# noegroup/bgflow

Hardware: AMD Instinct MI355X
Metric: flow samples/s (fwd+log|detJ|) at batch 2^20 (higher is better)
Workload: dtype f32 (split-f16 conditioner GEMMs: hi+lo f16 operand pairs, f32 accumulate)

## Files before the change

bgflow_amd/_lib.py:

```python
import ctypes
import os

import torch

_HERE = os.path.dirname(os.path.abspath(__file__))
LIB_PATH = os.environ.get("BGK_LIB") or os.path.join(_HERE, "libbgflow_amd.so")
_lib = None

i32, i64, f32, f64, vp = ctypes.c_int32, ctypes.c_int64, ctypes.c_float, ctypes.c_double, ctypes.c_void_p

_SIGNATURES = {
    "bgk_abi_version": (ctypes.c_int, []),
    "bgk_last_error": (ctypes.c_char_p, []),
    "bgk_set_option": (ctypes.c_int, [i32, i32]),
    "bgk_detmath_probe": (ctypes.c_int, [vp, i64, i32, vp, vp]),
    "bgk_rqs_transform": (ctypes.c_int, [vp, i64, vp, i64, i32, vp, i64, i32, i32, i32,
                                         f64, f64, f64, f64, f64, f64, f64, i32,
                                         vp, i64, vp, i32, vp, vp, vp]),
    "bgk_rqs_backward": (ctypes.c_int, [vp, i64, vp, i64, i32, vp, i64, i32, i32, i32,
                                        f64, f64, f64, f64, f64, f64, f64, i32,
                                        vp, i64, vp, vp, i64, vp, i64, vp, i32, vp]),
    "bgk_affine_transform": (ctypes.c_int, [vp, i64, vp, i64, vp, i64, vp, i32, i32, i32, i64, i32,
                                            vp, i64, vp, i32, vp]),
    "bgk_affine_backward": (ctypes.c_int, [vp, i64, vp, i64, vp, i64, vp, i32, i32, i32, i64, i32,
                                           vp, i64, vp, vp, i64, vp, i64, vp, i64, vp, vp, vp, vp]),
    "bgk_coupling_affine_dense_h2_train": (ctypes.c_int, [vp, vp, vp, i32, i32, vp, vp, vp, vp, i32, vp, vp, vp, vp, i32,
                                                          vp, i32, i32, i32, vp, i64, i64, i32, vp, i64, vp, i32,
                                                          vp, vp, vp, vp, i64, vp, vp, i64, vp]),
    "bgk_mlp_backward_dx": (ctypes.c_int, [vp, i64, i32, vp, vp, i64, vp, i64, i32, i32, vp, vp, vp, vp, i32, i64,
                                           vp, vp, vp, vp, vp, i64, vp, i64, vp, vp, vp]),
    "bgk_pack_mlp_h2": (ctypes.c_int, [vp, vp, i32, i32, vp, vp, i32, vp, vp, i32, vp, i32, i32, i32, vp, vp, vp, vp, vp]),
    "bgk_pack_mlp_h2_many": (ctypes.c_int, [i32] + [vp] * 18 + [vp]),
    "bgk_coupling_affine_dense_fwd64_train": (ctypes.c_int, [vp, i64, i32, vp, vp, vp, vp, i32, vp, vp, vp, vp, i32,
                                                             vp, i32, i32, i32, vp, i64, i64, i32, vp, i64, vp, i32,
                                                             vp, vp, vp, vp, vp, vp, i64, vp]),
    "bgk_pack_mlp_h2_t": (ctypes.c_int, [vp, i32, i32, vp, i32, vp, i32, vp, vp, vp, vp, vp]),
    "bgk_pack_mlp_h2_t_many": (ctypes.c_int, [i32] + [vp] * 11 + [vp]),
    "bgk_mlp_weight_grad_workspace": (i64, [i64, i32, i32, i32, i32]),
    "bgk_mlp_weight_grad": (ctypes.c_int, [vp, i64, i32, vp, vp, vp, vp, i64, i32, i32, i32, vp, i64, i32, i32, i64, vp, i64,
                                           vp, vp, vp, vp, vp, vp, i32, vp, vp]),
    "bgk_mlp_weight_grad_reduce_many": (ctypes.c_int, [i32] + [vp] * 12 + [i32, vp]),
    "bgk_ic_xyz2ic": (ctypes.c_int, [vp, i64, vp, i32, vp, i32, i32, f32, i32, vp, vp, i32, f32, i64,
                                     vp, vp, vp, i64, vp, i64, vp, i32, vp, vp]),
    "bgk_ic_ic2xyz": (ctypes.c_int, [vp, vp, vp, i64, vp, i64, vp, i32, vp, i32, i32, f32, i32,
                                     vp, vp, i32, f32, i64, vp, i64, vp, i32, vp, vp]),
    "bgk_ic_refsys": (ctypes.c_int, [vp, i64, i32, i32, f32, i32, vp, vp, i32, vp]),
    "bgk_icdf_ic2xyz": (ctypes.c_int, [vp, vp, vp, i64, vp, i64, vp, vp, vp, vp, i32, f32, vp, i32, vp, i32, i32, f32, i32,
                                       vp, vp, i32, f32, i64, vp, i64, vp, i32, vp, vp]),
    "bgk_icdf_ic2xyz_reg": (ctypes.c_int, [vp, vp, vp, vp, vp, i32, f32, vp, i32, vp, i32, f32, i32, vp, vp, i32, f64, i64,
                                           vp, i64, vp, i32, vp, vp]),
    "bgk_icdf_ic2xyz_uni": (ctypes.c_int, [vp, vp, vp, vp, vp, i32, f32, vp, i32, vp, i32, f32, i32, vp, vp, i32, f64, i64,
                                           vp, i64, vp, i32, vp, vp]),
    "bgk_icdf_ic2xyz_uni_train": (ctypes.c_int, [vp, vp, vp, vp, vp, i32, f32, vp, i32, vp, i32, f32, i32, vp, vp, i32, f64, i64,
                                                 vp, i64, vp, i32, vp, vp, vp, vp, vp, vp]),
    "bgk_icdf_ic2xyz_uni_train_kl": (ctypes.c_int, [vp, vp, vp, vp, vp, i32, f32, vp, i32, vp, i32, f32, i32, vp, vp, i32, f64, i64,
                                                    vp, i64, vp, vp, vp, vp, vp, vp, vp, f64, f64, f64, i32, vp, vp, vp, vp, vp]),
    "bgk_xyz2ic_cdf_uni": (ctypes.c_int, [vp, vp, i32, f32, vp, i32, vp, i32, f32, i32, vp, vp, i32, f64, i64,
                                          vp, vp, vp, vp, vp, i32, vp, vp]),
    "bgk_ic_ic2xyz_backward": (ctypes.c_int, [vp, vp, vp, i64, vp, i64, vp, i32, vp, i32, i32, f32, i32, vp, i32, i64,
                                              vp, i64, vp, vp, vp, vp, i64, vp, i64, vp, vp]),
    "bgk_cdf_transform": (ctypes.c_int, [vp, i64, vp, i64, i32, i32, i32, f32, vp, i64, vp, i32, vp]),
    "bgk_cdf_backward": (ctypes.c_int, [vp, i64, vp, i64, vp, i64, i32, i32, i32, f32, vp, i64, vp, vp, i64, vp]),
    "bgk_ic_xyz2ic_backward": (ctypes.c_int, [vp, i64, vp, i32, vp, i32, i32, f32, i32, vp, i32, i64,
                                              vp, vp, vp, i64, vp, i64, vp, vp, i64, vp]),
    "bgk_ic_refsys_backward": (ctypes.c_int, [vp, vp, vp, i64, i32, i32, f32, i32, vp, vp]),
    "bgk_coupling_rqs_dense": (ctypes.c_int, [vp, i64, i32, i32, vp, vp, vp, i32, i32, i32,
                                              vp, i64, i64, i32, i32, ctypes.c_uint64, i32,
                                              f64, f64, f64, f64, f64, f64, f64, i32,
                                              vp, i64, vp, i32, vp, vp, vp]),
    "bgk_coupling_rqs_dense_h2": (ctypes.c_int, [vp, i64, i32, i32, vp, vp, vp, f32, f32, f32, vp, i32, i32, i32, i32,
                                                 vp, i64, i64, i32, i32, ctypes.c_uint64, i32,
                                                 f64, f64, f64, f64, f64, f64, f64, i32,
                                                 vp, i64, vp, i32, vp, vp, vp]),
    "bgk_coupling_rqs_dense_deep": (ctypes.c_int, [vp, i64, i32, i32, vp, vp, vp, f32, vp, f32, i32, i32,
                                                   vp, i64, i64, i32, i32, ctypes.c_uint64, i32,
                                                   f64, f64, f64, f64, f64, f64, f64, i32,
                                                   vp, i64, vp, i32, vp, vp, vp]),
    "bgk_coupling_rqs_dense_h2_mc": (ctypes.c_int, [vp, vp, vp, i32, i32, vp, vp, vp, f32, f32, f32, vp, i32, i32, i32, i32,
                                                    vp, i64, i64, i32, i32, ctypes.c_uint64, i32,
                                                    f64, f64, f64, f64, f64, f64, f64, i32,
                                                    vp, i64, vp, i32, vp, vp, vp]),
    "bgk_coupling_affine_dense_h2_mc": (ctypes.c_int, [vp, vp, vp, i32, i32,
                                                       vp, vp, vp, f32, f32, f32, i32, vp, vp, vp, f32, f32, f32, i32,
                                                       i32, vp, i32, i32, i32, vp, i64, i64, i32, vp, i64, vp, i32, vp]),
    "bgk_coupling_affine_dense_h3_mc": (ctypes.c_int, [vp, vp, vp, i32, i32,
                                                       vp, vp, vp, vp, f32, f32, f32, f32, i32, vp, vp, vp, vp, f32, f32, f32, f32, i32,
                                                       i32, vp, i32, i32, i32, vp, i64, i64, i32, vp, i64, vp, i32, vp]),
    "bgk_pack_dense_h2": (ctypes.c_int, [vp, vp, i32, i32, vp, vp, vp, vp, i32, vp, i32, i32, i32, vp, vp, vp, vp, vp]),
    "bgk_coupling_rqs_dense_h2_train": (ctypes.c_int, [vp, i64, i32, i32, vp, vp, vp, f32, f32, f32, vp, i32, i32, i32,
                                                       vp, i64, i64, i32, i32, ctypes.c_uint64, i32,
                                                       f64, f64, f64, f64, f64, f64, f64, i32,
                                                       vp, i64, vp, i32, vp, vp, vp, vp, i64, vp, i32, vp]),
    "bgk_coupling_rqs_dense_h2_backward": (ctypes.c_int, [vp, vp, f32, vp, i32, i32, vp, i64, i64, i32, i32, i32, ctypes.c_uint64, i32,
                                                          f64, f64, f64, f64, f64, f64, f64, i32,
                                                          vp, i64, vp, vp, i64, vp, i64, vp, vp]),
    "bgk_coupling_affine_dense_h2": (ctypes.c_int, [vp, i64, i32, i32,
                                                    vp, vp, vp, f32, f32, f32, i32, vp, vp, vp, f32, f32, f32, i32,
                                                    i32, vp, i32, i32, i32, vp, i64, i64, i32, vp, i64, vp, i32, vp]),
    "bgk_coupling_affine_dense_h3": (ctypes.c_int, [vp, i64, i32, i32,
                                                    vp, vp, vp, vp, f32, f32, f32, f32, i32, vp, vp, vp, vp, f32, f32, f32, f32, i32,
                                                    i32, vp, i32, i32, i32, vp, i64, i64, i32, vp, i64, vp, i32, vp]),
    "bgk_coupling_affine_dense_deep": (ctypes.c_int, [vp, i64, i32, i32,
                                                      vp, vp, vp, f32, vp, f32, i32, vp, vp, vp, f32, vp, f32, i32,
                                                      i32, i32, vp, i32, i32, i32, vp, i64, i64, i32, vp, i64, vp, i32, vp]),
    "bgk_pack_dense_h2_t": (ctypes.c_int, [vp, i32, vp, vp, i32, vp, vp, vp, vp, vp]),
    "bgk_dense_backward_dx": (ctypes.c_int, [vp, i64, i32, vp, vp, vp, i64, i32, i32, vp, vp, vp, vp, i32, i64,
                                             vp, vp, vp, vp, vp, i64, vp, i64, vp, vp, vp]),
    "bgk_dense_weight_grad_reduce_many": (ctypes.c_int, [i32] + [vp] * 10 + [i32, vp]),
    "bgk_pack_dense_h2_many": (ctypes.c_int, [i32] + [vp] * 14 + [vp]),
    "bgk_pack_dense_h2_t_many": (ctypes.c_int, [i32] + [vp] * 9 + [vp]),
    "bgk_column_sum": (ctypes.c_int, [vp, i64, i64, i32, vp, i32, vp, vp]),
    "bgk_absmax": (ctypes.c_int, [vp, i64, i64, i32, vp, vp]),
    "bgk_whiten": (ctypes.c_int, [vp, i64, vp, vp, vp, i32, i32, i64, vp, i64, vp]),
    "bgk_normal_energy": (ctypes.c_int, [vp, i64, vp, i32, i64, f64, f64, vp, vp]),
    "bgk_normal_energy_backward": (ctypes.c_int, [vp, i64, vp, i32, i64, f64, vp, vp, i64, vp]),
    "bgk_energy_fields": (ctypes.c_int, [vp, vp, vp, vp, vp, vp, i32, i64, f64, f64, f64, vp, vp, i32, vp, i32, vp, vp]),
    "bgk_energy_fields_backward": (ctypes.c_int, [vp, vp, vp, vp, vp, vp, i32, i64, f64, vp, vp, vp, vp, i32, vp, vp, vp, vp]),
    "bgk_philox_fields": (ctypes.c_int, [ctypes.c_uint64, ctypes.c_uint32, i64, i32, vp, vp, vp, vp, vp, vp, vp, vp, f64, i64, vp, vp]),
    "bgk_colmap": (ctypes.c_int, [vp, i32, vp, i32, vp, vp, ctypes.c_uint64, ctypes.c_uint32, i64, i64, vp, i32, f64, vp, vp]),
    "bgk_grad_nan_flag":(ctypes.c_int, [vp, i64, vp, vp]),
    "bgk_adam_step": (ctypes.c_int, [vp, vp, vp, vp, i64, f32, f32, f32, f32, f32, i64, vp, vp, vp]),
    "bgk_dense_weight_grad_workspace": (i64, [i64, i32, i32]),
    "bgk_dense_weight_grad": (ctypes.c_int, [vp, i64, i32, vp, vp, vp, vp, i32, vp, i64, i32, i32, i64, vp, i64,
                                             vp, vp, vp, vp, vp, vp, i32, vp, vp]),
    "bgk_pack_rqs_columns": (i32, [i32, i32, vp, vp]),
    "bgk_dense_layer": (ctypes.c_int, [vp, i64, i64, i32, vp, i32, f32, vp, vp, i32, i32, vp, i64, i32, vp]),
    "bgk_pack_linear_layer": (ctypes.c_int, [vp, i64, i32, i32, vp, vp, vp]),
    "bgk_dense_layer_steps": (ctypes.c_int, [i32]),
    "bgk_refresh_linear_layer": (ctypes.c_int, [vp, i64, i32, i32, i32, vp, vp, vp, vp]),
    "bgk_activation": (ctypes.c_int, [vp, i64, i64, i32, i32, vp, i64, vp]),
    "bgk_activation_backward": (ctypes.c_int, [vp, i64, vp, i64, i64, i32, i32, vp, i64, vp]),
    "bgk_affine_net_backward64_workspace": (i64, [i64, i32, i32, i32, i32]),
    "bgk_affine_net_backward64": (ctypes.c_int, [vp, i64, i32, vp, vp, vp, i64, i32, i32, i32, vp, vp, vp, vp, i32, i64,
                                                 vp, i64, vp, i64, vp, vp, i64, vp, vp, vp, vp, vp, vp, i32, vp]),
    "bgk_affine_coupling_backward64_workspace": (i64, [i64, i32, i32, i32, i32, i32, i32]),
    "bgk_affine_coupling_backward64": (ctypes.c_int, [vp, i64, i32, vp, i64, i32, vp, i64, vp,
                                                      vp, vp, vp, vp, vp, i64,
                                                      vp, vp, vp, vp, vp, vp, i32, i32, i32,
                                                      vp, vp, vp, vp, vp, vp, vp, i32, i32, i32,
                                                      vp, i32, i64, vp, i64, vp, vp, i64, vp, i64, vp, vp, i64, vp, vp, i32, vp]),
    "bgk_linear_weight_grad_workspace": (i64, [i64, i32, i32]),
    "bgk_linear_weight_grad": (ctypes.c_int, [vp, i64, i32, vp, i64, i32, i64, vp, i64, vp, vp, i32, vp, vp]),
}

ABI_SYMBOLS = tuple(_SIGNATURES)


def lib():
    global _lib
    if _lib is None:
        if not os.path.exists(LIB_PATH):
            raise RuntimeError(
                f"{LIB_PATH} is missing: the MI355X kernels are not built. Run `python -m bgflow_amd.build` "
                "(hipcc, gfx950). bgflow_amd has no CPU fallback.")
        try:
            handle = ctypes.CDLL(LIB_PATH)
        except OSError as e:
            raise RuntimeError(f"cannot load {LIB_PATH}: {e}. bgflow_amd has no CPU fallback.") from e
        for name, (res, args) in _SIGNATURES.items():
            fn = getattr(handle, name)
            fn.restype = res
            fn.argtypes = args
        _lib = handle
    return _lib


def check(status, what):
    if status != 0:
        msg = lib().bgk_last_error().decode(errors="replace")
        if status == -1 and "Minimal bin" in msg:
            raise ValueError(msg)
        raise RuntimeError(f"{what} failed (status {status}): {msg}")


def require_hip(*tensors):
    for t in tensors:
        if t is None:
            continue
        if not t.is_cuda:
            raise RuntimeError(
                "bgflow_amd kernels run on MI355X (HIP) tensors only; got a tensor on "
                f"'{t.device}'. There is no CPU fallback in this package.")
        if t.dtype not in (torch.float32, torch.int32):
            raise RuntimeError(f"bgflow_amd kernels are float32; got {t.dtype}")


def ptr(t):
    return None if t is None else ctypes.c_void_p(t.data_ptr())


def cond_segments(parts):
    rows = [rowmajor(t) for t in parts]
    n = len(rows)
    ptrs = (ctypes.c_void_p * n)(*[t.data_ptr() for t, _ in rows])
    lds = (ctypes.c_int64 * n)(*[ld for _, ld in rows])
    widths = (ctypes.c_int32 * n)(*[t.shape[1] for t, _ in rows])
    return ptrs, lds, widths, n, rows


def stream_ptr(device=None):
    return ctypes.c_void_p(torch.cuda.current_stream(device).cuda_stream)


def rowmajor(t):
    assert t.dim() == 2, "expected [batch, features]"
    if t.stride(1) != 1 and t.shape[1] > 1:
        t = t.contiguous()
    if t.shape[1] == 1 and t.stride(1) != 1:
        t = t.contiguous()
    ld = t.stride(0) if t.shape[0] > 1 else t.shape[1]
    if t.shape[0] > 1 and ld < t.shape[1]:
        t = t.contiguous()
        ld = t.stride(0)
    return t, ld
```

bgflow_amd/csrc/bgk_capi.hip:

```cpp
#include <stdarg.h>

#include "bgk_common.h"
#include "bgk_fused2.h"

extern int bgk_affine_variant;

static thread_local char g_err[512] = "";

void bgk_set_error(const char* fmt, ...) {
    va_list ap;
    va_start(ap, fmt);
    vsnprintf(g_err, sizeof(g_err), fmt, ap);
    va_end(ap);
}

extern "C" int bgk_abi_version(void) { return 1; }
extern "C" const char* bgk_last_error(void) { return g_err; }

extern "C" int bgk_set_option(int32_t option, int32_t value) {
    if (option == 1 && (value == 1 || value == 2)) {
        const int prev = bgk_h2_variant;
        bgk_h2_variant = value;
        return prev;
    }
    if (option == 2 && (value == 1 || value == 2)) {
        const int prev = bgk_affine_variant;
        bgk_affine_variant = value;
        return prev;
    }
    if (option == 3 && (value == 1 || value == 2)) {
        const int prev = bgk_rc_vjp_variant;
        bgk_rc_vjp_variant = value;
        return prev;
    }
    bgk_set_error("bgk_set_option: unknown option %d / value %d", option, value);
    return BGK_EINVAL;
}

namespace {
__global__ void detmath_probe_kernel(const float* x, int64_t n, int which, float* out) {
    int64_t i = (int64_t)blockIdx.x * blockDim.x + threadIdx.x;
    if (i >= n) return;
    float v = x[i], r;
    switch (which) {
        case 0: r = bgk_expf(v); break;
        case 1: r = bgk_logf(v); break;
        case 2: r = bgk_softplusf(v, 0.69384102162f); break;
        case 3: r = bgk_siluf(v); break;
        case 4: r = bgk_tanhf(v); break;
        default: r = v;
    }
    out[i] = r;
}
}

extern "C" int bgk_detmath_probe(const float* x, int64_t n, int32_t which, float* out, void* stream) {
    if (n <= 0) return 0;
    int grid = (int)((n + 255) / 256);
    hipLaunchKernelGGL(detmath_probe_kernel, dim3(grid), dim3(256), 0, (hipStream_t)stream, x, n, which, out);
    return bgk_launch_status("bgk_detmath_probe");
}
```

bgflow_amd/csrc/bgk_fused2.h:

```cpp
#ifndef BGK_FUSED2_H
#define BGK_FUSED2_H
#include <stdint.h>

#define BGK_MAX_COND 3
struct BgkCondSegs { const float* ptr[BGK_MAX_COND]; int64_t ld[BGK_MAX_COND]; int32_t w[BGK_MAX_COND]; int32_t n; };

int bgk_launch_rqs_dense_h2v2(const char* what, const float* cond, int64_t ldc, int32_t d_c, int32_t periodic,
                              const void* A0p, const void* A1p, const void* A2p, float c0, float c1, float c2, const float* cs_dev,
                              int32_t act, const float* y, int64_t ldy, int64_t B, int32_t d, uint64_t circ_mask, int32_t inverse,
                              double left, double right, double bottom, double top,
                              double min_bin_width, double min_bin_height, double min_derivative, int32_t identity_init,
                              float* out, int64_t ldo, float* dlogp, int32_t accumulate, int32_t* bin_idx, int32_t* oob_count,
                              void* stream, const BgkCondSegs* segs = nullptr);

int bgk_launch_rqs_dense_h2v2_train(const char* what, float* z0, float* z1, float* params, int64_t ldp, const int32_t* src_col,
                                    const float* cond, int64_t ldc, int32_t d_c, int32_t periodic,
                                    const void* A0p, const void* A1p, const void* A2p, float c0, float c1, float c2, const float* cs_dev,
                                    int32_t act, const float* y, int64_t ldy, int64_t B, int32_t d, uint64_t circ_mask, int32_t inverse,
                                    double left, double right, double bottom, double top,
                                    double min_bin_width, double min_bin_height, double min_derivative, int32_t identity_init,
                                    float* out, int64_t ldo, float* dlogp, int32_t accumulate, int32_t* bin_idx, int32_t* oob_count,
                                    void* stream, const BgkCondSegs* segs = nullptr);

int bgk_launch_rqs_bwd_recompute(const char* what, const float* z1, const void* A2p, float c2, const float* cs_dev, int32_t act,
                                 const float* y, int64_t ldy, int64_t B, int32_t d, uint64_t circ_mask, int32_t inverse,
                                 double left, double right, double bottom, double top,
                                 double min_bin_width, double min_bin_height, double min_derivative, int32_t identity_init,
                                 const float* g_out, int64_t ldgo, const float* g_dlogp, float* g_y, int64_t ldgy,
                                 float* g_params, int64_t ldgp, float* g_absmax, void* stream);

int bgk_launch_rqs_dense_h2v2_bf16(const char* what, const float* cond, int64_t ldc, int32_t d_c, int32_t periodic,
                                   const void* A0p, const void* A1p, const void* A2p, float c0, float c1, float c2, const float* cs_dev,
                                   int32_t act, const float* y, int64_t ldy, int64_t B, int32_t d, uint64_t circ_mask, int32_t inverse,
                                   double left, double right, double bottom, double top,
                                   double min_bin_width, double min_bin_height, double min_derivative, int32_t identity_init,
                                   float* out, int64_t ldo, float* dlogp, int32_t accumulate, int32_t* bin_idx, int32_t* oob_count,
                                   void* stream, const BgkCondSegs* segs = nullptr);

int bgk_launch_affine_dense_v2(const float* cond, int64_t ldc, int32_t d_c, int32_t periodic,
                               const void* sA0, const void* sA1, const void* sA1b, const void* sA2, float sc0, float sc1, float sc1b, float sc2, int32_t s_act,
                               const void* tA0, const void* tA1, const void* tA1b, const void* tA2, float tc0, float tc1, float tc1b, float tc2, int32_t t_act,
                               const float* log_alpha, int32_t preserve_volume, int32_t is_circular, int32_t inverse,
                               const float* y, int64_t ldy, int64_t B, int32_t d,
                               float* out, int64_t ldo, float* dlogp, int32_t accumulate, void* stream, const BgkCondSegs* segs = nullptr);

struct BgkAffTrainSave { const float* s_cs; float* s_z0; float* s_z1; const float* t_cs; float* t_z0; float* t_z1; float* mu; float* s_raw; int64_t ldms;
                         int64_t ldz; };
int bgk_launch_affine_dense_v2_train(const BgkAffTrainSave* save, const float* cond, int64_t ldc, int32_t d_c, int32_t periodic,
                               const void* sA0, const void* sA1, const void* sA1b, const void* sA2, float sc0, float sc1, float sc1b, float sc2, int32_t s_act,
                               const void* tA0, const void* tA1, const void* tA1b, const void* tA2, float tc0, float tc1, float tc1b, float tc2, int32_t t_act,
                               const float* log_alpha, int32_t preserve_volume, int32_t is_circular, int32_t inverse,
                               const float* y, int64_t ldy, int64_t B, int32_t d,
                               float* out, int64_t ldo, float* dlogp, int32_t accumulate, void* stream, const BgkCondSegs* segs = nullptr);

extern int bgk_h2_variant;
extern int bgk_rc_vjp_variant;

#endif
```

bgflow_amd/csrc/bgk_fused2.hip:

```cpp
#include "bgk_common.h"
#include "bgk_fused2.h"

#ifndef BGK_V2_SAVE
#define BGK_V2_SAVE 0
#endif
#if BGK_V2_SAVE
#include "bgk_mfma_h2.h"
#include "bgk_rqs_vjp.h"
#define coupling_rqs_dense_h2v2_kernel coupling_rqs_dense_h2v2_train_kernel
#endif
#ifndef BGK_V2_BF16
#define BGK_V2_BF16 0
#endif
#if BGK_V2_BF16
#define coupling_rqs_dense_h2v2_kernel coupling_rqs_dense_h2v2_bf16_kernel
typedef short s16x8 __attribute__((ext_vector_type(8)));
#endif
#ifndef BGK_V2_AFFTRAIN
#define BGK_V2_AFFTRAIN 0
#endif
#if BGK_V2_AFFTRAIN
#define coupling_affine_dense_v2_kernel coupling_affine_dense_v2_train_kernel
#endif
constexpr int NPROD = BGK_V2_BF16 ? 1 : 3;

namespace {

typedef float f32x16 __attribute__((ext_vector_type(16)));
typedef _Float16 h16x8 __attribute__((ext_vector_type(8)));
typedef unsigned u32x4 __attribute__((ext_vector_type(4)));

constexpr int FW = 4;
constexpr int FTHREADS = FW * 64;
constexpr int KB = 8;
constexpr int PPD = 3 * KB + 1;
constexpr int DPC = 128 / PPD;
constexpr int SROW = 33;
constexpr int ST = BGK_V2_SAVE ? 33 : 32;
constexpr int KS = 8;
constexpr int GBLK = KS * 8 + 4;
#ifndef BGK_V2_KARG
#define BGK_V2_KARG 2
#endif
#ifndef BGK_V2_RD
#define BGK_V2_RD 4
#endif
#ifndef BGK_V2_TS
#define BGK_V2_TS 0
#endif
#if BGK_V2_TS
#define V2_TS(k) do { const unsigned long long t_ = __builtin_amdgcn_s_memtime(); if (lane == 0 && a.bin_idx) a.bin_idx[b0 * d + (k)] = (int)(unsigned)t_; } while (0)
#else
#define V2_TS(k) do { } while (0)
#endif
constexpr int RD = BGK_V2_RD;
constexpr int EH = 34;

struct CondSegs {
    const float* ptr[BGK_MAX_COND]; int64_t ld[BGK_MAX_COND]; int w[BGK_MAX_COND]; int off[BGK_MAX_COND]; uint32_t magic[BGK_MAX_COND];
    int n;
};

struct SetK { float gnum, low, high, dstep; float kc[7]; };

struct SpC {
    float left, right;
    SetK sa, sb;
    float beta, kout, min_d;
};

struct V2Args {
    CondSegs cs;
    int d_c; int periodic;
    const float* y; int64_t ldy; float* out; int64_t ldo; int d; uint32_t magic_d;
    int64_t B; float* dlogp; int accumulate; int32_t* bin_idx; int32_t* oob_count;
    const uint4* A0; const uint4* A1; const uint4* A2; int S0; int n_chunks; int last_tiles;
    float c0, c1, c2; const float* cs_dev;
    uint64_t circ_mask;
    SpC sc;
    int lds_per_wave;
    int nfs, ys, stage, y_dma, out_lin;
#if BGK_V2_SAVE
    float* z0; float* z1;
    float* params; int64_t ldp;
    const int32_t* src_col;
#endif
};
typedef const __attribute__((address_space(4))) V2Args* kargs_t;

struct BFrag { h16x8 hi[KS], lo[KS]; };
struct TFrag { u32x4 hi, lo; };

__device__ __forceinline__ int drow(int m, int r, int hh) { return 32 * m + (r & 3) + 8 * (r >> 2) + 4 * hh; }

template <int NT, int MS = 4, int RDX = RD>
struct Live {
    static constexpr int NTS = KS * NT;
    static constexpr int NEV = NPROD * NTS + NT;
    f32x16 (&out)[4];
    const BFrag& b;
    const uint4* W;
    unsigned voff;
    TFrag (&ring)[RDX];
    __amdgpu_buffer_rsrc_t rs;

    template <int BLK>
    __device__ __forceinline__ u32x4 blk() {
        return __builtin_amdgcn_raw_buffer_load_b128(rs, voff + ((BLK * 1024) & 4095), (BLK * 1024) & ~4095, 0);
    }
    template <int T>
    __device__ __forceinline__ void load() {
        if constexpr (T < NTS) {
            constexpr int s = T / NT, m = T % NT;
#if BGK_V2_BF16
            ring[T % RDX].hi = blk<(s * MS + m) * 2>();
#else
            ring[T % RDX].hi = blk<(s * MS + m) * 2>();
            ring[T % RDX].lo = blk<(s * MS + m) * 2 + 1>();
#endif
        } else if constexpr (T < NTS + NT) {
            ring[T % RDX].hi = blk<KS * MS * 2 + (T - NTS)>();
        }
    }
    template <int T0, int T1>
    __device__ __forceinline__ void loads() {
        if constexpr (T0 < T1) { load<T0>(); loads<T0 + 1, T1>(); }
    }
    __device__ __forceinline__ void start() {
        __builtin_amdgcn_sched_barrier(0);
        rs = __builtin_amdgcn_make_buffer_rsrc((void*)W, 0, 0x7fffffff, 0x00020000);
        loads<0, RDX>();
        __builtin_amdgcn_sched_barrier(0);
    }
    template <int E>
    __device__ __forceinline__ void event() {
        __builtin_amdgcn_sched_barrier(0);
#if BGK_V2_BF16
        if constexpr (E < NTS) {
            constexpr int T = E, s = T / NT, m = T % NT;
            const s16x8 a = __builtin_bit_cast(s16x8, ring[T % RDX].hi), bb = __builtin_bit_cast(s16x8, b.hi[s]);
            if constexpr (s == 0) {
                const f32x16 z = {0.f, 0.f, 0.f, 0.f, 0.f, 0.f, 0.f, 0.f, 0.f, 0.f, 0.f, 0.f, 0.f, 0.f, 0.f, 0.f};
                out[m] = __builtin_amdgcn_mfma_f32_32x32x16_bf16(a, bb, z, 0, 0, 0);
            } else {
                out[m] = __builtin_amdgcn_mfma_f32_32x32x16_bf16(a, bb, out[m], 0, 0, 0);
            }
            load<T + RDX>();
        } else if constexpr (E < NEV) {
            constexpr int m = E - NTS, T = NTS + m;
            const s16x8 one2 = {(short)0x3f80, (short)0x3f80, 0, 0, 0, 0, 0, 0};
            out[m] = __builtin_amdgcn_mfma_f32_32x32x16_bf16(__builtin_bit_cast(s16x8, ring[T % RDX].hi), one2, out[m], 0, 0, 0);
        }
#else
        if constexpr (E < 3 * NTS) {
            constexpr int T = E / 3, p = E % 3, s = T / NT, m = T % NT;
            const TFrag& f = ring[T % RDX];
            const h16x8 a = __builtin_bit_cast(h16x8, p == 0 ? f.lo : f.hi);
            const h16x8 bb = p == 1 ? b.lo[s] : b.hi[s];
            if constexpr (s == 0 && p == 0) {
                const f32x16 z = {0.f, 0.f, 0.f, 0.f, 0.f, 0.f, 0.f, 0.f, 0.f, 0.f, 0.f, 0.f, 0.f, 0.f, 0.f, 0.f};
                out[m] = __builtin_amdgcn_mfma_f32_32x32x16_f16(a, bb, z, 0, 0, 0);
            } else {
                out[m] = __builtin_amdgcn_mfma_f32_32x32x16_f16(a, bb, out[m], 0, 0, 0);
            }
            if constexpr (p == 2) load<T + RDX>();
        } else if constexpr (E < NEV) {
            constexpr int m = E - 3 * NTS, T = NTS + m;
            const h16x8 one2 = {(_Float16)1.0f, (_Float16)1.0f, 0, 0, 0, 0, 0, 0};
            out[m] = __builtin_amdgcn_mfma_f32_32x32x16_f16(__builtin_bit_cast(h16x8, ring[T % RDX].hi), one2, out[m], 0, 0, 0);
        }
#endif
        __builtin_amdgcn_sched_barrier(0);
    }
    template <int E0, int E1>
    __device__ __forceinline__ void events() {
        if constexpr (E0 < E1) {
            event<E0>();
            events<E0 + 1, E1>();
        }
    }
    template <int HK, int NH>
    __device__ __forceinline__ void hook() {
        constexpr int e0 = (HK * NEV) / NH, e1 = ((HK + 1) * NEV) / NH;
        if constexpr (e0 < e1) events<e0, e1>();
    }
};
struct NoLive {
    template <int HK, int NH> __device__ __forceinline__ void hook() {}
};

template <class G, int BASE, int NH>
struct Hooks {
    G& g;
    template <int I> __device__ __forceinline__ void at() { g.template hook<BASE + I, NH>(); }
};

template <int ACT, int T, int P, class H>
__device__ __forceinline__ void act_split_pair(H& hk, const f32x16& t, float c, BFrag& bf) {
    constexpr int r = 2 * P;
    float a0, a1;
    if constexpr (ACT == 2) {
        a0 = t[r] * c; a1 = t[r + 1] * c;
        hk.template at<3 * P>();
        a0 = a0 > 0.0f ? a0 : 0.0f; a1 = a1 > 0.0f ? a1 : 0.0f;
        hk.template at<3 * P + 1>();
    } else {
        constexpr float kk = ACT == 1 ? -1.44269504088896341f : 2.88539008177792681f;
        const float ck = c * kk, rc = 1.0f / c;
        const float e0 = __builtin_amdgcn_exp2f(t[r] * ck), e1 = __builtin_amdgcn_exp2f(t[r + 1] * ck);
        hk.template at<3 * P>();
        if constexpr (ACT == 1) {
            const float q0 = __builtin_amdgcn_rcpf(__builtin_fmaf(e0, rc, rc)), q1 = __builtin_amdgcn_rcpf(__builtin_fmaf(e1, rc, rc));
            a0 = t[r] * q0; a1 = t[r + 1] * q1;
        } else {
            const float q0 = __builtin_amdgcn_rcpf(1.0f + e0), q1 = __builtin_amdgcn_rcpf(1.0f + e1);
            a0 = 1.0f - 2.0f * q0; a1 = 1.0f - 2.0f * q1;
        }
        hk.template at<3 * P + 1>();
    }
    constexpr int s = 2 * T + (r >> 3), e = r & 7;
#if BGK_V2_BF16
    typedef __bf16 bf2v __attribute__((ext_vector_type(2)));
    typedef float f2v __attribute__((ext_vector_type(2)));
    typedef _Float16 h2v __attribute__((ext_vector_type(2)));
    const bf2v pb = __builtin_convertvector((f2v){a0, a1}, bf2v);
    const h2v ph = __builtin_bit_cast(h2v, pb);
    bf.hi[s][e] = ph[0]; bf.hi[s][e + 1] = ph[1];
#else
    unsigned uh, ul;
    asm("v_cvt_pk_f16_f32 %0, %1, %2" : "=v"(uh) : "v"(a0), "v"(a1));
    asm("v_fma_mixlo_f16 %0, %1, -1.0, %2 op_sel:[0,0,0] op_sel_hi:[1,0,0]" : "=v"(ul) : "v"(uh), "v"(a0));
    asm("v_fma_mixhi_f16 %0, %1, -1.0, %2 op_sel:[1,0,0] op_sel_hi:[1,0,0]" : "+v"(ul) : "v"(uh), "v"(a1));
    typedef _Float16 h2v __attribute__((ext_vector_type(2)));
    const h2v ph = __builtin_bit_cast(h2v, uh), pl = __builtin_bit_cast(h2v, ul);
    bf.hi[s][e] = ph[0]; bf.hi[s][e + 1] = ph[1];
    bf.lo[s][e] = pl[0]; bf.lo[s][e + 1] = pl[1];
#endif
    hk.template at<3 * P + 2>();
}
template <int ACT, int T, class H>
__device__ __forceinline__ void act_split_tile(H hk, const f32x16& t, float c, BFrag& bf) {
    act_split_pair<ACT, T, 0>(hk, t, c, bf); act_split_pair<ACT, T, 1>(hk, t, c, bf);
    act_split_pair<ACT, T, 2>(hk, t, c, bf); act_split_pair<ACT, T, 3>(hk, t, c, bf);
    act_split_pair<ACT, T, 4>(hk, t, c, bf); act_split_pair<ACT, T, 5>(hk, t, c, bf);
    act_split_pair<ACT, T, 6>(hk, t, c, bf); act_split_pair<ACT, T, 7>(hk, t, c, bf);
}

struct SpK { float kL, kz, c2; };

__device__ __forceinline__ float fdiv_hw(float n, float d) {
    const float r = __builtin_amdgcn_rcpf(d);
    const float q = n * r;
    return __builtin_fmaf(__builtin_fmaf(-d, q, n), r, q);
}
__device__ __forceinline__ float rcp_nr(float d) {
    const float r = __builtin_amdgcn_rcpf(d);
    return __builtin_fmaf(__builtin_fmaf(-d, r, 1.0f), r, r);
}

template <bool KARG> struct ScSrc;
template <> struct ScSrc<true> {
    kargs_t ka;
    __device__ __forceinline__ ScSrc(const V2Args&) { ka = (kargs_t)__builtin_amdgcn_kernarg_segment_ptr(); asm volatile("" : "+s"(ka)); }
    __device__ __forceinline__ const __attribute__((address_space(4))) SpC& get() const { return ka->sc; }
};
template <> struct ScSrc<false> {
    const V2Args& a;
    __device__ __forceinline__ ScSrc(const V2Args& a_) : a(a_) {}
    __device__ __forceinline__ const SpC& get() const { return a.sc; }
};

template <int INV, class H>
__device__ __forceinline__ float rqs_fast(H hk, float x, const float* pa, const float* pb, const float* ps, bool circ,
                                          const V2Args& a, const SpK& k, float* lad, int* bin, int* oob) {
    const ScSrc<(BGK_V2_KARG == 2 ? INV != 0 : BGK_V2_KARG != 0)> scs(a);
#define SC scs.get()
    float va[KB], vb[KB];
#pragma unroll
    for (int i = 0; i < KB; ++i) va[i] = pa[i * ST];
#pragma unroll
    for (int i = 0; i < KB; ++i) vb[i] = pb[i * ST];
    *oob = (x < SC.left) | (x > SC.right);
    x = __builtin_amdgcn_fmed3f(x, SC.left, SC.right);
    float mA = __builtin_fmaxf(__builtin_fmaxf(va[0], va[1]), va[2]);
    mA = __builtin_fmaxf(__builtin_fmaxf(mA, va[3]), va[4]);
    mA = __builtin_fmaxf(__builtin_fmaxf(mA, va[5]), va[6]);
    mA = __builtin_fmaxf(mA, va[7]);
    const float nmA = -(mA * k.kL);
    hk.template at<0>();
    float E[KB];
    E[0] = __builtin_amdgcn_exp2f(__builtin_fmaf(va[0], k.kL, nmA));
    E[1] = __builtin_amdgcn_exp2f(__builtin_fmaf(va[1], k.kL, nmA));
    E[2] = __builtin_amdgcn_exp2f(__builtin_fmaf(va[2], k.kL, nmA));
    hk.template at<1>();
    E[3] = __builtin_amdgcn_exp2f(__builtin_fmaf(va[3], k.kL, nmA));
    E[4] = __builtin_amdgcn_exp2f(__builtin_fmaf(va[4], k.kL, nmA));
    E[5] = __builtin_amdgcn_exp2f(__builtin_fmaf(va[5], k.kL, nmA));
    hk.template at<2>();
    E[6] = __builtin_amdgcn_exp2f(__builtin_fmaf(va[6], k.kL, nmA));
    E[7] = __builtin_amdgcn_exp2f(__builtin_fmaf(va[7], k.kL, nmA));
    E[1] += E[0]; E[2] += E[1];
    hk.template at<3>();
    E[3] += E[2]; E[4] += E[3]; E[5] += E[4]; E[6] += E[5]; E[7] += E[6];
    hk.template at<4>();
    const float gA = SC.sa.gnum * rcp_nr(E[7]);
    float kn[7];
    kn[0] = __builtin_fmaf(E[0], gA, SC.sa.kc[0]);
    kn[1] = __builtin_fmaf(E[1], gA, SC.sa.kc[1]);
    hk.template at<5>();
    kn[2] = __builtin_fmaf(E[2], gA, SC.sa.kc[2]);
    kn[3] = __builtin_fmaf(E[3], gA, SC.sa.kc[3]);
    kn[4] = __builtin_fmaf(E[4], gA, SC.sa.kc[4]);
    kn[5] = __builtin_fmaf(E[5], gA, SC.sa.kc[5]);
    kn[6] = __builtin_fmaf(E[6], gA, SC.sa.kc[6]);
    hk.template at<6>();
    float low_a = SC.sa.low, high_a = SC.sa.high;
    asm volatile("" : "+s"(low_a), "+s"(high_a));
#pragma unroll
    for (int i = 0; i < 7; ++i) asm volatile("" : "+v"(kn[i]));
    const bool g3 = x >= kn[3];
    hk.template at<7>();
    float w0 = g3 ? kn[3] : low_a, w1 = g3 ? kn[4] : kn[0], w2 = g3 ? kn[5] : kn[1], w3 = g3 ? kn[6] : kn[2];
    hk.template at<8>();
    float w4 = g3 ? high_a : kn[3];
    const bool gm = x >= w2;
    const float v0 = gm ? w2 : w0, v1 = gm ? w3 : w1, v2 = gm ? w4 : w2;
    hk.template at<9>();
    const bool gl = x >= v1;
    const float lo = gl ? v1 : v0, hi = gl ? v2 : v1;
    float idxf = g3 ? 4.0f : 0.0f;
    hk.template at<10>();
    idxf += gm ? 2.0f : 0.0f;
    idxf += gl ? 1.0f : 0.0f;
    const int idx = (int)idxf;
    *bin = idx;
    hk.template at<11>();
    const int j1 = circ ? ((idx + 1) & 7) : (idx + 1);
    const float s_lo = ps[idx * ST], s_hi = ps[j1 * ST];
    const float A_i = hi - lo;
    float mB = __builtin_fmaxf(__builtin_fmaxf(vb[0], vb[1]), vb[2]);
    hk.template at<12>();
    mB = __builtin_fmaxf(__builtin_fmaxf(mB, vb[3]), vb[4]);
    mB = __builtin_fmaxf(__builtin_fmaxf(mB, vb[5]), vb[6]);
    mB = __builtin_fmaxf(mB, vb[7]);
    const float nmB = -(mB * k.kL);
    float F[KB];
    F[0] = __builtin_amdgcn_exp2f(__builtin_fmaf(vb[0], k.kL, nmB));
    hk.template at<13>();
    F[1] = __builtin_amdgcn_exp2f(__builtin_fmaf(vb[1], k.kL, nmB));
    F[2] = __builtin_amdgcn_exp2f(__builtin_fmaf(vb[2], k.kL, nmB));
    F[3] = __builtin_amdgcn_exp2f(__builtin_fmaf(vb[3], k.kL, nmB));
    hk.template at<14>();
    F[4] = __builtin_amdgcn_exp2f(__builtin_fmaf(vb[4], k.kL, nmB));
    F[5] = __builtin_amdgcn_exp2f(__builtin_fmaf(vb[5], k.kL, nmB));
    F[6] = __builtin_amdgcn_exp2f(__builtin_fmaf(vb[6], k.kL, nmB));
    hk.template at<15>();
    F[7] = __builtin_amdgcn_exp2f(__builtin_fmaf(vb[7], k.kL, nmB));
    F[1] += F[0]; F[2] += F[1]; F[3] += F[2];
    hk.template at<16>();
    F[4] += F[3]; F[5] += F[4]; F[6] += F[5]; F[7] += F[6];
    const float rB = __builtin_amdgcn_rcpf(F[7]);
    hk.template at<17>();
    const float gB = SC.sb.gnum * __builtin_fmaf(__builtin_fmaf(-F[7], rB, 1.0f), rB, rB);
    const float f0 = g3 ? F[3] : 0.0f, f1 = g3 ? F[4] : F[0], f2 = g3 ? F[5] : F[1];
    hk.template at<18>();
    const float f3 = g3 ? F[6] : F[2], f4 = g3 ? F[7] : F[3];
    const float u0 = gm ? f2 : f0, u1 = gm ? f3 : f1, u2 = gm ? f4 : f2;
    hk.template at<19>();
    const float Flo = gl ? u1 : u0;
    float Fhi = gl ? u2 : u1;
    hk.template at<20>();
    const float cb = __builtin_fmaf(idxf, SC.sb.dstep, SC.sb.low);
    hk.template at<21>();
    const float b_i = __builtin_fmaf(Flo, gB, cb);
    float b_ip1 = __builtin_fmaf(Fhi, gB, cb + SC.sb.dstep);
    float top_b = SC.sb.high;
    asm volatile("" : "+s"(top_b));
    b_ip1 = (g3 && gm && gl) ? top_b : b_ip1;
    const float B_i = b_ip1 - b_i;
    const float z0 = s_lo * k.kz;
    hk.template at<22>();
    const float ez0 = __builtin_amdgcn_exp2f(z0);
    float lg0 = __builtin_amdgcn_logf(1.0f + ez0);
    asm volatile("" : "+v"(lg0));
    const float sm0 = ez0 * __builtin_fmaf(ez0, -0.5f, 1.0f) * 1.44269504088896341f;
    hk.template at<23>();
    float l0 = (ez0 < 2.44140625e-4f ? sm0 : lg0) * SC.kout;
    asm volatile("" : "+v"(l0));
    l0 = z0 > 28.8539008177792681f ? s_lo * k.c2 : l0;
    const float d_i = SC.min_d + l0;
    const float z1 = s_hi * k.kz;
    hk.template at<24>();
    const float ez1 = __builtin_amdgcn_exp2f(z1);
    float lg1 = __builtin_amdgcn_logf(1.0f + ez1);
    asm volatile("" : "+v"(lg1));
    const float sm1 = ez1 * __builtin_fmaf(ez1, -0.5f, 1.0f) * 1.44269504088896341f;
    hk.template at<25>();
    float l1 = (ez1 < 2.44140625e-4f ? sm1 : lg1) * SC.kout;
    asm volatile("" : "+v"(l1));
    l1 = z1 > 28.8539008177792681f ? s_hi * k.c2 : l1;
    const float d_ip1 = SC.min_d + l1;
    float cw_i, W_i, ch_i, H_i;
    if (INV) { cw_i = lo; W_i = A_i; ch_i = b_i; H_i = B_i; }
    else { ch_i = lo; H_i = A_i; cw_i = b_i; W_i = B_i; }
    hk.template at<26>();
    const float delta = fdiv_hw(H_i, W_i);
    const float S = d_i + d_ip1 - 2.0f * delta;
    hk.template at<27>();
    float outv, l;
    if (!INV) {
        const float dx = x - ch_i;
        const float dxS = dx * S;
        const float qa = dxS + H_i * (delta - d_i);
        const float qb = H_i * d_i - dxS;
        hk.template at<28>();
        const float qc = -delta * dx;
        const float disc = qb * qb - 4.0f * qa * qc;
        const float sq = __builtin_amdgcn_sqrtf(disc);
        hk.template at<29>();
        const float root = fdiv_hw(2.0f * qc, -qb - sq);
        outv = __builtin_fmaf(root, W_i, cw_i);
        hk.template at<30>();
        const float omr = 1.0f - root;
        const float t1mt = root * omr;
        const float den = delta + S * t1mt;
        const float lden = __builtin_amdgcn_logf(den);
        hk.template at<31>();
        const float num = (delta * delta) * (d_ip1 * (root * root) + 2.0f * delta * t1mt + d_i * (omr * omr));
        hk.template at<32>();
        l = (2.0f * lden - __builtin_amdgcn_logf(num)) * 0.693147180559945309f;
    } else {
        const float theta = fdiv_hw(x - cw_i, W_i);
        const float omt = 1.0f - theta;
        hk.template at<28>();
        const float t1mt = theta * omt;
        const float numer = H_i * (delta * (theta * theta) + d_i * t1mt);
        const float den = delta + S * t1mt;
        hk.template at<29>();
        outv = ch_i + fdiv_hw(numer, den);
        const float lden = __builtin_amdgcn_logf(den);
        hk.template at<30>();
        const float inner = d_ip1 * (theta * theta) + 2.0f * delta * t1mt;
        hk.template at<31>();
        const float num = (delta * delta) * (inner + d_i * (omt * omt));
        hk.template at<32>();
        l = (__builtin_amdgcn_logf(num) - 2.0f * lden) * 0.693147180559945309f;
    }
    hk.template at<33>();
    *lad = l;
    return outv;
}

#undef SC

template <int INV, int IT, int NHK, class G>
__device__ __forceinline__ void spline_slot(G& g, const V2Args& a, const SpK& k, const float* s_p, float* s_y, int c, int nd,
                                            int hh, int j, int rows, float& run, int& oob_local, int (&bins)[3]) {
    const int q = 2 * IT + hh;
    const bool valid = q < nd;
    const int qq = valid ? q : 0;
    const int dim = c * DPC + qq;
    const float* pw = s_p + (qq * PPD) * ST + j;
    const float* ph = pw + KB * ST;
    const float* ps = ph + KB * ST;
    const bool circ = (a.circ_mask >> dim) & 1ull;
    int bin, oob;
    float lad;
    const float x = s_y[j * a.ys + dim];
    Hooks<G, IT * EH, NHK> hk{g};
    const float o = rqs_fast<INV>(hk, x, INV ? pw : ph, INV ? ph : pw, ps, circ, a, k, &lad, &bin, &oob);
    s_y[valid ? j * a.ys + dim : 32 * a.ys + j] = o;
    oob_local += (valid && j < rows) ? oob : 0;
    bins[IT] = bin;
    lad = valid ? lad : 0.0f;
    float l0 = lad, l1 = lad;
    asm volatile("s_nop 1\n\tv_permlane32_swap_b32 %0, %1" : "+v"(l0), "+v"(l1));
    run += l0;
    run += l1;
}

__device__ __forceinline__ void chunk_to_lds(const f32x16 (&h)[4], float* s_p, int hh, int j) {
#pragma unroll
    for (int m = 0; m < 4; ++m)
#pragma unroll
        for (int r = 0; r < 16; ++r) s_p[drow(m, r, hh) * ST + j] = h[m][r];
    __builtin_amdgcn_fence(__ATOMIC_ACQ_REL, "wavefront");
    __builtin_amdgcn_wave_barrier();
}

#if BGK_V2_SAVE
__device__ __forceinline__ void save_chunk_params(const V2Args& a, const float* s_p, int c, int lane, int64_t b0, int rows) {
    if (a.params == nullptr) return;
    if (a.src_col == nullptr) {
        typedef float f4s __attribute__((ext_vector_type(4), aligned(4)));
        const int l = lane & 31, half = lane >> 5;
        const int nd = (a.d - c * DPC) < DPC ? (a.d - c * DPC) : DPC;
        const bool mine = 4 * l < nd * PPD;
        for (int jj = 0; jj < rows; jj += 2) {
            const int r = jj + half;
            if (r < rows && mine) {
                float* prow = a.params + (b0 + r) * a.ldp + (DPC * PPD) * c;
                const f4s v = {s_p[(4 * l) * ST + r] * a.c2, s_p[(4 * l + 1) * ST + r] * a.c2, s_p[(4 * l + 2) * ST + r] * a.c2, s_p[(4 * l + 3) * ST + r] * a.c2};
                *reinterpret_cast<f4s*>(prow + 4 * l) = v;
            }
        }
        return;
    }
    const int col_lo = a.src_col[c * 128 + lane], col_hi = a.src_col[c * 128 + 64 + lane];
    for (int jj = 0; jj < rows; ++jj) {
        float* prow = a.params + (b0 + jj) * a.ldp;
        if (col_lo >= 0) prow[col_lo] = s_p[lane * ST + jj] * a.c2;
        if (col_hi >= 0) prow[col_hi] = s_p[(64 + lane) * ST + jj] * a.c2;
    }
}
#endif

template <int INV, int NT, bool SAVEP>
__device__ __forceinline__ void chunk_piped(const V2Args& a, const SpK& k, float* s_p, float* s_y, int c, int hh, int j, int rows,
                                            float& run, int& oob_local, int (&bins)[3], f32x16 (&h)[4], const BFrag& bf,
                                            TFrag (&ring)[RD], unsigned voff, int64_t b0) {
    Live<NT> g{h, bf, a.A2 + (size_t)(c + 1) * GBLK * 64, voff, ring};
    g.start();
    chunk_to_lds(h, s_p, hh, j);
#if BGK_V2_SAVE
    if constexpr (SAVEP) save_chunk_params(a, s_p, c, (int)threadIdx.x & 63, b0, rows);
#endif
    __builtin_amdgcn_sched_barrier(0);
    spline_slot<INV, 0, 3 * EH>(g, a, k, s_p, s_y, c, DPC, hh, j, rows, run, oob_local, bins);
    spline_slot<INV, 1, 3 * EH>(g, a, k, s_p, s_y, c, DPC, hh, j, rows, run, oob_local, bins);
    spline_slot<INV, 2, 3 * EH>(g, a, k, s_p, s_y, c, DPC, hh, j, rows, run, oob_local, bins);
}

typedef const __attribute__((address_space(1))) void* gvp_t;
typedef __attribute__((address_space(3))) void* lvp_t;
__device__ __forceinline__ void dma_tile32(float* dst, const float* __restrict__ src, int n, int valid, int lane) {
    for (int c = 0; c < n; c += 256) {
        const int e = c + lane * 4;
        if (e + 3 < valid) __builtin_amdgcn_global_load_lds((gvp_t)(src + e), (lvp_t)(dst + c), 16, 0, 0);
    }
    if (valid & 3) {
        const int edge = valid & ~3;
        if (lane < (valid & 3)) __builtin_amdgcn_global_load_lds((gvp_t)(src + edge + lane), (lvp_t)(dst + edge), 4, 0, 0);
    }
}

__device__ __forceinline__ void v2_sincos2pi(float x, float* s, float* c) {
    const float f = __builtin_amdgcn_fractf(x);
    *s = __builtin_amdgcn_sinf(f);
    *c = __builtin_amdgcn_cosf(f);
}

struct StageTiles { int d_c, periodic, nfs, ys, stage, y_dma, d; uint32_t magic_d; int rows, lane; };

__device__ __forceinline__ void stage_issue(const StageTiles& t, const CondSegs& cs, int64_t b0, const float* y_t, float* s_p, float* s_y) {
    if (t.y_dma) dma_tile32(s_y, y_t, 32 * t.d, t.rows * t.d, t.lane);
    if (t.stage == 1) dma_tile32(s_p, cs.ptr[0] + b0 * cs.ld[0], 32 * t.d_c, t.rows * t.d_c, t.lane);
    else if (t.stage == 2) dma_tile32(s_p + 32 * t.nfs, cs.ptr[0] + b0 * cs.ld[0], 32 * t.d_c, t.rows * t.d_c, t.lane);
}

#ifndef BGK_V2_SB
#define BGK_V2_SB 8
#endif
template <class KA>
__device__ __forceinline__ void stage_finish(const StageTiles& t, const CondSegs& cs, int64_t b0, const float* y_t, int ldy32,
                                             float* s_p, float* s_y, float y_fill) {
    constexpr int SB = BGK_V2_SB;
    const int lane = t.lane, rows = t.rows, d = t.d, nfs = t.nfs, n_y = 32 * t.d;
    if (!t.y_dma) {
        for (int base = 0; base < n_y; base += 64 * SB) {
            float vy[SB];
#pragma unroll
            for (int u = 0; u < SB; ++u) {
                const int i = base + u * 64 + lane;
                const int r = (int)(__umul24((unsigned)i, t.magic_d) >> 20), c = i - (int)__umul24((unsigned)r, (unsigned)d);
                vy[u] = (i < n_y && r < rows) ? y_t[(int)__umul24((unsigned)r, (unsigned)ldy32) + c] : y_fill;
            }
#pragma unroll
            for (int u = 0; u < SB; ++u) {
                const int i = base + u * 64 + lane;
                const int r = (int)(__umul24((unsigned)i, t.magic_d) >> 20), c = i - (int)__umul24((unsigned)r, (unsigned)d);
                if (i < n_y) s_y[(int)__umul24((unsigned)r, (unsigned)t.ys) + c] = vy[u];
            }
        }
    }
    if (t.stage == 0) {
        typedef const __attribute__((address_space(4))) KA* ka_t;
        const ka_t kseg = (ka_t)__builtin_amdgcn_kernarg_segment_ptr();
        for (int sg = 0; sg < cs.n; ++sg) {
            const float* cond_t = kseg->cs.ptr[sg] + b0 * kseg->cs.ld[sg];
            const int ldc32 = (int)kseg->cs.ld[sg], w_c = kseg->cs.w[sg], n_c = 32 * w_c, col0 = kseg->cs.off[sg];
            const uint32_t magic_c = kseg->cs.magic[sg];
            for (int base = 0; base < n_c; base += 64 * SB) {
                float vc[SB];
#pragma unroll
                for (int u = 0; u < SB; ++u) {
                    const int i = base + u * 64 + lane;
                    const int r = (int)(__umul24((unsigned)i, magic_c) >> 20), c = i - (int)__umul24((unsigned)r, (unsigned)w_c);
                    vc[u] = (i < n_c && r < rows) ? cond_t[(int)__umul24((unsigned)r, (unsigned)ldc32) + c] : 0.0f;
                }
#pragma unroll
                for (int u = 0; u < SB; ++u) {
                    const int i = base + u * 64 + lane;
                    const int r = (int)(__umul24((unsigned)i, magic_c) >> 20), c = i - (int)__umul24((unsigned)r, (unsigned)w_c);
                    if (i < n_c) {
                        float* f = s_p + (int)__umul24((unsigned)r, (unsigned)nfs) + col0 + c;
                        if (t.periodic) {
                            float sv, cv;
                            v2_sincos2pi(vc[u], &sv, &cv);
                            f[0] = cv;
                            f[t.d_c] = sv;
                        } else {
                            f[0] = vc[u];
                        }
                    }
                }
            }
        }
    }
    asm volatile("s_waitcnt vmcnt(0)" ::: "memory");
    __builtin_amdgcn_fence(__ATOMIC_ACQ_REL, "wavefront");
    __builtin_amdgcn_wave_barrier();
    if (t.stage == 2) {
        const float* raw = s_p + 32 * nfs;
        const uint32_t magic_c = cs.magic[0];
        for (int i = lane; i < 32 * t.d_c; i += 64) {
            const int r = (int)(__umul24((unsigned)i, magic_c) >> 20), c = i - (int)__umul24((unsigned)r, (unsigned)t.d_c);
            float sv, cv;
            v2_sincos2pi(raw[i], &sv, &cv);
            float* f = s_p + (int)__umul24((unsigned)r, (unsigned)nfs) + c;
            f[0] = cv;
            f[t.d_c] = sv;
        }
    }
    if (t.stage != 1) {
        __builtin_amdgcn_fence(__ATOMIC_ACQ_REL, "wavefront");
        __builtin_amdgcn_wave_barrier();
    }
}

__device__ __forceinline__ void store_tile32(float* out_t, int ldo32, const float* s_y, int ys, int d, uint32_t magic_d, int rows, int lane, int lin) {
    const int n = rows * d;
    if (lin) {
        for (int i = lane * 4; i + 3 < n; i += 256) *reinterpret_cast<float4*>(out_t + i) = *reinterpret_cast<const float4*>(s_y + i);
        if (lane < (n & 3)) out_t[(n & ~3) + lane] = s_y[(n & ~3) + lane];
    } else {
        for (int i = lane; i < n; i += 64) {
            const int r = (int)(__umul24((unsigned)i, magic_d) >> 20), cc = i - (int)__umul24((unsigned)r, (unsigned)d);
            out_t[(int)__umul24((unsigned)r, (unsigned)ldo32) + cc] = s_y[(int)__umul24((unsigned)r, (unsigned)ys) + cc];
        }
    }
}

struct L0Frag { uint4 v[4][2]; };
__device__ __forceinline__ void l0_request(L0Frag& f, const uint4* A0, int s, int lane) {
#pragma unroll
    for (int m = 0; m < 4; ++m) {
        f.v[m][0] = A0[((s * 4 + m) * 2 + 0) * 64 + lane];
#if !BGK_V2_BF16
        f.v[m][1] = A0[((s * 4 + m) * 2 + 1) * 64 + lane];
#endif
    }
}
__device__ __forceinline__ void l0_step(f32x16 (&h)[4], const L0Frag& fr, const float* f, bool last, int rel0) {
    float v[8];
#pragma unroll
    for (int e = 0; e < 8; ++e) v[e] = f[e];
    if (last) {
#pragma unroll
        for (int e = 0; e < 8; ++e) v[e] = rel0 + e == 0 ? 1.0f : (rel0 + e > 0 ? 0.0f : v[e]);
    }
#if BGK_V2_BF16
    s16x8 bb;
#pragma unroll
    for (int e = 0; e < 8; ++e) bb[e] = __builtin_bit_cast(short, (__bf16)v[e]);
#pragma unroll
    for (int m = 0; m < 4; ++m)
        h[m] = __builtin_amdgcn_mfma_f32_32x32x16_bf16(__builtin_bit_cast(s16x8, fr.v[m][0]), bb, h[m], 0, 0, 0);
#else
    h16x8 bhi, blo;
#pragma unroll
    for (int e = 0; e < 8; ++e) {
        const float c = v[e];
        const _Float16 hv = (_Float16)c;
        bhi[e] = hv;
        blo[e] = (_Float16)(c - (float)hv);
    }
#pragma unroll
    for (int m = 0; m < 4; ++m) h[m] = __builtin_amdgcn_mfma_f32_32x32x16_f16(__builtin_bit_cast(h16x8, fr.v[m][1]), bhi, h[m], 0, 0, 0);
#pragma unroll
    for (int m = 0; m < 4; ++m) h[m] = __builtin_amdgcn_mfma_f32_32x32x16_f16(__builtin_bit_cast(h16x8, fr.v[m][0]), blo, h[m], 0, 0, 0);
#pragma unroll
    for (int m = 0; m < 4; ++m) h[m] = __builtin_amdgcn_mfma_f32_32x32x16_f16(__builtin_bit_cast(h16x8, fr.v[m][0]), bhi, h[m], 0, 0, 0);
#endif
}

template <int ACT, int INV, bool SAVEP = true>
__global__ __launch_bounds__(FTHREADS, 2) void coupling_rqs_dense_h2v2_kernel(V2Args a) {
    if (a.cs_dev) { a.c0 = a.cs_dev[1]; a.c1 = a.cs_dev[3]; a.c2 = a.cs_dev[5]; }
    asm volatile("s_setreg_imm32_b32 hwreg(HW_REG_MODE, 23, 1), 1");
    extern __shared__ __attribute__((aligned(16))) float smem[];
    const int wave = threadIdx.x >> 6;
    float* s_p = smem + (size_t)wave * a.lds_per_wave;
    float* s_y = s_p + 128 * ST;
    const int d = a.d;
    const int64_t n_tiles = (a.B + 31) / 32;
    const int64_t tile = (int64_t)blockIdx.x * FW + wave;
    if (tile >= n_tiles) return;
    const SpK k{a.c2 * 1.44269504088896341f, a.c2 * a.sc.beta * 1.44269504088896341f, a.c2};
    const int n_in = a.periodic ? 2 * a.d_c : a.d_c;
    const int ldy32 = (int)a.ldy, ldo32 = (int)a.ldo;
    const int n_y = 32 * d;

  {
    const int lane = (int)threadIdx.x & 63, j = lane & 31, hh = lane >> 5;
    const unsigned voff = (unsigned)lane * 16u;
    const int64_t b0 = tile * 32;
    const int rows = (int)((a.B - b0) < 32 ? (a.B - b0) : 32);
    const float* y_t = a.y + b0 * a.ldy;
    float* out_t = a.out + b0 * a.ldo;
    V2_TS(0);

    const int nfs = a.nfs, ys = a.ys;
    const StageTiles stg{a.d_c, a.periodic, nfs, ys, a.stage, a.y_dma, d, a.magic_d, rows, lane};
    stage_issue(stg, a.cs, b0, y_t, s_p, s_y);
    f32x16 h[4], acc[4];
    TFrag ring[RD];
    BFrag bf;
    L0Frag fa, fb;
    l0_request(fa, a.A0, 0, lane);
    Live<4> g1{acc, bf, a.A1, voff, ring};
    g1.start();
    V2_TS(12);
    stage_finish<V2Args>(stg, a.cs, b0, y_t, ldy32, s_p, s_y, 0.5f);
    V2_TS(1);

#pragma unroll
    for (int m = 0; m < 4; ++m)
#pragma unroll
        for (int r = 0; r < 16; ++r) h[m][r] = 0.0f;
    {
        const float* frow = s_p + j * nfs + 8 * hh;
        const int rel0 = 16 * (a.S0 - 1) + 8 * hh - n_in;
        for (int s = 0; s < a.S0; s += 2) {
            if (s + 1 < a.S0) l0_request(fb, a.A0, s + 1, lane);
            l0_step(h, fa, frow + 16 * s, s + 1 == a.S0, rel0);
            if (s + 1 < a.S0) {
                if (s + 2 < a.S0) l0_request(fa, a.A0, s + 2, lane);
                l0_step(h, fb, frow + 16 * (s + 1), s + 2 == a.S0, rel0);
            }
        }
    }

    V2_TS(2);
    {
        Live<4>& g = g1;
#if BGK_V2_SAVE
#pragma unroll
        for (int m = 0; m < 4; ++m)
#pragma unroll
            for (int r = 0; r < 16; ++r) h[m][r] *= a.c0;
        h2_store_rows128(h, a.z0, s_p, b0, rows, lane);
        const float c0_act = 1.0f;
#else
        const float c0_act = a.c0;
#endif
        NoLive none;
        act_split_tile<ACT, 0>(Hooks<NoLive, 0, 1>{none}, h[0], c0_act, bf);
        __builtin_amdgcn_sched_barrier(0);
        V2_TS(14);
        act_split_tile<ACT, 1>(Hooks<Live<4>, 0, 100>{g}, h[1], c0_act, bf);
        act_split_tile<ACT, 2>(Hooks<Live<4>, 24, 100>{g}, h[2], c0_act, bf);
        act_split_tile<ACT, 3>(Hooks<Live<4>, 48, 100>{g}, h[3], c0_act, bf);
        __builtin_amdgcn_sched_barrier(0);
        V2_TS(15);
        g.template events<(72 * Live<4>::NEV) / 100, Live<4>::NEV>();
    }

    V2_TS(3);
    float run = 0.0f;
    int oob_local = 0;
    {
        Live<4> g{h, bf, a.A2, voff, ring};
        g.start();
#if BGK_V2_SAVE
#pragma unroll
        for (int m = 0; m < 4; ++m)
#pragma unroll
            for (int r = 0; r < 16; ++r) acc[m][r] *= a.c1;
        h2_store_rows128(acc, a.z1, s_p, b0, rows, lane);
        const float c1_act = 1.0f;
#else
        const float c1_act = a.c1;
#endif
        NoLive none;
        act_split_tile<ACT, 0>(Hooks<NoLive, 0, 1>{none}, acc[0], c1_act, bf);
        __builtin_amdgcn_sched_barrier(0);
        act_split_tile<ACT, 1>(Hooks<Live<4>, 0, 100>{g}, acc[1], c1_act, bf);
        act_split_tile<ACT, 2>(Hooks<Live<4>, 24, 100>{g}, acc[2], c1_act, bf);
        act_split_tile<ACT, 3>(Hooks<Live<4>, 48, 100>{g}, acc[3], c1_act, bf);
        __builtin_amdgcn_sched_barrier(0);
        g.template events<(72 * Live<4>::NEV) / 100, Live<4>::NEV>();
    }
    V2_TS(4);
    for (int c = 0; c < a.n_chunks; ++c) {
        int bins[3] = {0, 0, 0};
        const int nd = (d - c * DPC) < DPC ? (d - c * DPC) : DPC;
        if (c + 2 < a.n_chunks || (c + 2 == a.n_chunks && a.last_tiles > 2)) {
            chunk_piped<INV, 4, SAVEP>(a, k, s_p, s_y, c, hh, j, rows, run, oob_local, bins, h, bf, ring, voff, b0);
        } else if (c + 2 == a.n_chunks) {
            chunk_piped<INV, 2, SAVEP>(a, k, s_p, s_y, c, hh, j, rows, run, oob_local, bins, h, bf, ring, voff, b0);
        } else {
            NoLive none;
            chunk_to_lds(h, s_p, hh, j);
#if BGK_V2_SAVE
            if constexpr (SAVEP) save_chunk_params(a, s_p, c, lane, b0, rows);
#endif
            spline_slot<INV, 0, 1>(none, a, k, s_p, s_y, c, nd, hh, j, rows, run, oob_local, bins);
            if (nd > 2) spline_slot<INV, 1, 1>(none, a, k, s_p, s_y, c, nd, hh, j, rows, run, oob_local, bins);
            if (nd > 4) spline_slot<INV, 2, 1>(none, a, k, s_p, s_y, c, nd, hh, j, rows, run, oob_local, bins);
        }
#if BGK_V2_TS
        V2_TS(5 + c);
#else
        if (a.bin_idx) {
#pragma unroll
            for (int it = 0; it < 3; ++it) {
                const int q = 2 * it + hh;
                if (q < nd && j < rows) a.bin_idx[(b0 + j) * d + c * DPC + q] = bins[it];
            }
        }
#endif
        __builtin_amdgcn_fence(__ATOMIC_ACQ_REL, "wavefront");
        __builtin_amdgcn_wave_barrier();
    }
    if (hh == 0 && j < rows) {
        if (a.accumulate) a.dlogp[b0 + j] += run; else a.dlogp[b0 + j] = run;
    }
    store_tile32(out_t, ldo32, s_y, ys, d, a.magic_d, rows, lane, a.out_lin);
    if (a.oob_count && __builtin_amdgcn_ballot_w64(oob_local != 0)) {
        for (int off = 32; off > 0; off >>= 1) oob_local += __shfl_xor(oob_local, off);
        if (lane == 0) atomicAdd(a.oob_count, oob_local);
    }
    V2_TS(5 + a.n_chunks);
  }
}

struct TilePlan { int nfs, ys, stage, y_dma, out_lin; };
TilePlan plan_tiles(const CondSegs& cs, int d_c, int periodic, const float* y, int64_t ldy, const float* out, int64_t ldo, int d, int tile_floats) {
    const int n_in = periodic ? 2 * d_c : d_c;
    const auto dma_ok = [](const float* p, int64_t ld, int w) { return ld == w && ((uintptr_t)p & 15) == 0 && (w & 7) != 0; };
    TilePlan t;
    t.y_dma = dma_ok(y, ldy, d) ? 1 : 0;
    t.ys = t.y_dma ? d : (d | 1);
    t.out_lin = (t.y_dma && ldo == d && ((uintptr_t)out & 15) == 0) ? 1 : 0;
    const bool c_dma = cs.n == 1 && dma_ok(cs.ptr[0], cs.ld[0], d_c);
    t.stage = (c_dma && !periodic) ? 1 : ((c_dma && periodic && 32 * ((n_in | 1) + d_c) <= tile_floats) ? 2 : 0);
    t.nfs = t.stage == 1 ? d_c : (n_in | 1);
    return t;
}

SetK make_set(double low, double high, double min_bin, int K) {
    SetK s;
    const double span = high - low, scale = 1.0 - min_bin * K;
    s.gnum = (float)((double)(float)span * (double)(float)scale);
    s.low = (float)low; s.high = (float)high;
    s.dstep = (float)((double)(float)span * (double)(float)min_bin);
    for (int k = 0; k < 7; ++k) s.kc[k] = (float)((double)(float)low + (double)(float)span * (double)(float)min_bin * (k + 1));
    return s;
}

uint32_t magic_div(int d) { return (uint32_t)(((1u << 20) + (uint32_t)d - 1) / (uint32_t)d); }

bool make_cond_segs(CondSegs& cs, const float* cond, int64_t ldc, int d_c, const BgkCondSegs* segs) {
    for (int i = 0; i < BGK_MAX_COND; ++i) { cs.ptr[i] = nullptr; cs.ld[i] = 0; cs.w[i] = 0; cs.off[i] = 0; cs.magic[i] = 0; }
    if (!segs || segs->n <= 1) {
        const float* p = segs && segs->n == 1 ? segs->ptr[0] : cond;
        const int64_t ld = segs && segs->n == 1 ? segs->ld[0] : ldc;
        if (!p || d_c <= 0 || ld >= (1 << 24)) return false;
        cs.n = 1; cs.ptr[0] = p; cs.ld[0] = ld; cs.w[0] = d_c; cs.magic[0] = magic_div(d_c);
        return true;
    }
    if (segs->n > BGK_MAX_COND) return false;
    int off = 0;
    for (int i = 0; i < segs->n; ++i) {
        if (!segs->ptr[i] || segs->w[i] <= 0 || segs->ld[i] < segs->w[i] || segs->ld[i] >= (1 << 24)) return false;
        cs.ptr[i] = segs->ptr[i]; cs.ld[i] = segs->ld[i]; cs.w[i] = segs->w[i]; cs.off[i] = off; cs.magic[i] = magic_div(segs->w[i]);
        off += segs->w[i];
    }
    cs.n = segs->n;
    return off == d_c;
}


#if !BGK_V2_SAVE && !BGK_V2_BF16
struct AffV2Net { const uint4* A0; const uint4* A1; const uint4* A1b; const uint4* A2; float c0, c1, c1b, c2;
#if BGK_V2_AFFTRAIN
                  const float* cs;
                  float* z0; float* z1;
#endif
};
struct AffV2Args {
    CondSegs cs; int d_c; int periodic; int S0;
    AffV2Net shift, scale; int has_shift, has_scale;
    const float* log_alpha; int preserve_volume, is_circular, inverse;
    const float* y; int64_t ldy; int64_t B; int d;
    float* out; int64_t ldo; float* dlogp; int accumulate;
    uint32_t magic_d;
    int lds_tile, lds_per_wave;
    int nfs, ys, stage, y_dma, out_lin;
#if BGK_V2_AFFTRAIN
    float* mu_out; float* s_out; int64_t ldms;
    int slab;
    int zt;
#endif
};

#if BGK_V2_AFFTRAIN
template <int NT>
__device__ __forceinline__ void aff_store_tiles(const f32x16 (&t)[4], float* dst, int pitch, float* slab, int64_t b0, int rows, int lane) {
    const int j = lane & 31, hh = lane >> 5;
    const __amdgpu_buffer_rsrc_t rs = __builtin_amdgcn_make_buffer_rsrc((void*)(dst + b0 * pitch), 0, rows * pitch * 4, 0x00020000);
#pragma unroll
    for (int m = 0; m < NT; ++m)
#pragma unroll
        for (int half = 0; half < 2; ++half) {
            if ((j >> 4) == half) {
#pragma unroll
                for (int q = 0; q < 4; ++q)
                    *reinterpret_cast<float4*>(slab + (j & 15) * 32 + 4 * ((2 * q + hh) ^ (j & 7))) =
                        make_float4(t[m][4 * q], t[m][4 * q + 1], t[m][4 * q + 2], t[m][4 * q + 3]);
            }
            __builtin_amdgcn_fence(__ATOMIC_ACQ_REL, "wavefront");
            __builtin_amdgcn_wave_barrier();
#pragma unroll
            for (int it = 0; it < 2; ++it) {
                const int i = it * 64 + lane, r = i >> 3, p = i & 7;
                const float4 v = *reinterpret_cast<const float4*>(slab + r * 32 + 4 * (p ^ (r & 7)));
                __builtin_amdgcn_raw_buffer_store_b128(__builtin_bit_cast(u32x4, v), rs, ((16 * half + r) * pitch + 32 * m + 4 * p) * 4, 0, 0);
            }
            __builtin_amdgcn_fence(__ATOMIC_ACQ_REL, "wavefront");
            __builtin_amdgcn_wave_barrier();
        }
}
struct AffSave { float* slab; int64_t b0; int rows, lane, zt; };
#endif

__device__ __forceinline__ void aff_layer0(const AffV2Net& n, int S0, const float* s_p, int nfs, int n_in, int lane, int j, int hh,
                                           f32x16 (&X)[4], L0Frag& fa, bool requested) {
    L0Frag fb;
    if (!requested) l0_request(fa, n.A0, 0, lane);
#pragma unroll
    for (int m = 0; m < 4; ++m)
#pragma unroll
        for (int r = 0; r < 16; ++r) X[m][r] = 0.0f;
    const float* frow = s_p + j * nfs + 8 * hh;
    const int rel0 = 16 * (S0 - 1) + 8 * hh - n_in;
    for (int s = 0; s < S0; s += 2) {
        if (s + 1 < S0) l0_request(fb, n.A0, s + 1, lane);
        l0_step(X, fa, frow + 16 * s, s + 1 == S0, rel0);
        if (s + 1 < S0) {
            if (s + 2 < S0) l0_request(fa, n.A0, s + 2, lane);
            l0_step(X, fb, frow + 16 * (s + 1), s + 2 == S0, rel0);
        }
    }
}

#if BGK_V2_AFFTRAIN
#define AFF_SAVE_PARAMS , float* zdst, const AffSave& sv
#define AFF_SAVE_Z(X) do { _Pragma("unroll") for (int m_ = 0; m_ < 4; ++m_) _Pragma("unroll") for (int r_ = 0; r_ < 16; ++r_) X[m_][r_] *= c; \
                           if (sv.zt == 2) aff_store_tiles<2>(X, zdst, 64, sv.slab, sv.b0, sv.rows, sv.lane); \
                           else aff_store_tiles<4>(X, zdst, 128, sv.slab, sv.b0, sv.rows, sv.lane); \
                           c = 1.0f; } while (0)
#else
#define AFF_SAVE_PARAMS
#define AFF_SAVE_Z(X) do { } while (0)
#endif
template <int ACT>
__device__ __forceinline__ void aff_hidden(const uint4* A, float c, f32x16 (&X)[4], f32x16 (&Y)[4], BFrag& bf, TFrag (&ring)[RD], unsigned voff AFF_SAVE_PARAMS) {
    NoLive none;
    Live<4> g{Y, bf, A, voff, ring};
    g.start();
    AFF_SAVE_Z(X);
    act_split_tile<ACT, 0>(Hooks<NoLive, 0, 1>{none}, X[0], c, bf);
    __builtin_amdgcn_sched_barrier(0);
    act_split_tile<ACT, 1>(Hooks<Live<4>, 0, 100>{g}, X[1], c, bf);
    act_split_tile<ACT, 2>(Hooks<Live<4>, 24, 100>{g}, X[2], c, bf);
    act_split_tile<ACT, 3>(Hooks<Live<4>, 48, 100>{g}, X[3], c, bf);
    __builtin_amdgcn_sched_barrier(0);
    g.template events<(72 * Live<4>::NEV) / 100, Live<4>::NEV>();
}
template <int ACT, int OT>
__device__ __forceinline__ void aff_output(const uint4* A, float c, f32x16 (&X)[4], f32x16 (&Y)[4], BFrag& bf, TFrag (&ring)[RD], unsigned voff AFF_SAVE_PARAMS) {
    NoLive none;
    typedef Live<OT, OT> GO;
    GO g{Y, bf, A, voff, ring};
    g.start();
    AFF_SAVE_Z(X);
    act_split_tile<ACT, 0>(Hooks<NoLive, 0, 1>{none}, X[0], c, bf);
// ... 357 lines not shown
    {
        f32x16 z[4];
#pragma unroll
        for (int m = 0; m < 4; ++m)
#pragma unroll
            for (int q = 0; q < 4; ++q) {
                const int piece = (8 * m + 2 * q + hh) ^ (j & 15);
                const float4 v = *reinterpret_cast<const float4*>(s_p + j * 128 + piece * 4);
                z[m][4 * q] = v.x; z[m][4 * q + 1] = v.y; z[m][4 * q + 2] = v.z; z[m][4 * q + 3] = v.w;
            }
        NoLive none;
        act_split_tile<ACT, 0>(Hooks<NoLive, 0, 1>{none}, z[0], 1.0f, bf);
        act_split_tile<ACT, 1>(Hooks<NoLive, 0, 1>{none}, z[1], 1.0f, bf);
        act_split_tile<ACT, 2>(Hooks<NoLive, 0, 1>{none}, z[2], 1.0f, bf);
        act_split_tile<ACT, 3>(Hooks<NoLive, 0, 1>{none}, z[3], 1.0f, bf);
    }
    __builtin_amdgcn_fence(__ATOMIC_ACQ_REL, "wavefront");
    __builtin_amdgcn_wave_barrier();
    RC_Q(q2);
    g0.template events<0, Live<4, 4, RC_RD>::NEV>();
    RC_Q(q3);
    const int jr = j < rows ? j : rows - 1;
    const float gl = (a.g_dlogp + b0)[jr];
    float gmax = 0.0f;
    const RcTile tl{__builtin_amdgcn_make_buffer_rsrc((void*)(a.y + b0 * a.ldy), 0, (int)(rows * a.ldy * 4), 0x00020000),
                    __builtin_amdgcn_make_buffer_rsrc((void*)(a.g_out + b0 * a.ldgo), 0, (int)(rows * a.ldgo * 4), 0x00020000),
                    __builtin_amdgcn_make_buffer_rsrc((void*)(a.g_y + b0 * a.ldgy), 0, (int)(rows * a.ldgy * 4), 0x00020000),
                    __builtin_amdgcn_make_buffer_rsrc((void*)(a.g_params + b0 * a.ldgp), 0, (int)(rows * a.ldgp * 4), 0x00020000),
                    jr * (int)a.ldy * 4, jr * (int)a.ldgo * 4, j * (int)a.ldgy * 4};
    RcIn in = rc_request(tl, 0, 0, a.d < DPC ? a.d : DPC, hh);
    for (int c = 0; c + 1 < a.n_chunks; ++c) {
        if (c + 2 < a.n_chunks || a.last_tiles > 2) rc_chunk<4, 3, FAST>(a, tl, s_p, c, DPC, lane, rows, gl, gmax, in, h, bf, ring, voff, ts);
        else rc_chunk<2, 3, FAST>(a, tl, s_p, c, DPC, lane, rows, gl, gmax, in, h, bf, ring, voff, ts);
    }
    {
        const int c = a.n_chunks - 1, nd = a.d - c * DPC;
        if (nd > 4) rc_chunk<0, 3, FAST>(a, tl, s_p, c, nd, lane, rows, gl, gmax, in, h, bf, ring, voff, ts);
        else if (nd > 2) rc_chunk<0, 2, FAST>(a, tl, s_p, c, nd, lane, rows, gl, gmax, in, h, bf, ring, voff, ts);
        else rc_chunk<0, 1, FAST>(a, tl, s_p, c, nd, lane, rows, gl, gmax, in, h, bf, ring, voff, ts);
    }
    bgk_publish_absmax(a.g_absmax, gmax);
#if BGK_RC_TS
    asm volatile("s_waitcnt vmcnt(0)" ::: "memory");
    unsigned q4;
    RC_Q(q4);
    if (lane == 0) {
        unsigned* o = reinterpret_cast<unsigned*>(a.g_y + b0 * a.ldgy);
        o[0] = q1 - q0; o[1] = q2 - q1; o[2] = q3 - q2; o[3] = ts.lds; o[4] = ts.vjp; o[5] = ts.gemm; o[6] = ts.st; o[7] = q4 - q0;
    }
#endif
}
#endif

}

#if !BGK_V2_SAVE && !BGK_V2_BF16 && !BGK_V2_AFFTRAIN
int bgk_h2_variant = 2;
#endif

#if BGK_V2_SAVE
int bgk_rc_vjp_variant = 2;
int bgk_launch_rqs_bwd_recompute(const char* what, const float* z1, const void* A2p, float c2, const float* cs_dev, int32_t act,
                                 const float* y, int64_t ldy, int64_t B, int32_t d, uint64_t circ_mask, int32_t inverse,
                                 double left, double right, double bottom, double top,
                                 double min_bin_width, double min_bin_height, double min_derivative, int32_t identity_init,
                                 const float* g_out, int64_t ldgo, const float* g_dlogp, float* g_y, int64_t ldgy,
                                 float* g_params, int64_t ldgp, float* g_absmax, void* stream) {
    RcArgs a;
    a.z1 = z1; a.A2 = reinterpret_cast<const uint4*>(A2p); a.c2 = c2; a.cs_dev = cs_dev;
    a.n_chunks = (d + DPC - 1) / DPC;
    a.last_tiles = ((d - (a.n_chunks - 1) * DPC) * PPD + 31) / 32;
    a.y = y; a.ldy = ldy; a.B = B; a.d = d; a.nc_mask = ~circ_mask & (d >= 64 ? ~0ull : ((1ull << d) - 1ull)); a.inverse = inverse;
    BGK_CHECK_ARG(ldy < (1 << 24) && ldgo < (1 << 24) && ldgy < (1 << 24) && ldgp < (1 << 24), "%s: row stride too large", what);
    a.g_out = g_out; a.ldgo = ldgo; a.g_dlogp = g_dlogp; a.g_y = g_y; a.ldgy = ldgy; a.g_params = g_params; a.ldgp = ldgp;
    a.g_absmax = g_absmax;
    a.cfg = bgk_make_rqs_cfg(left, right, bottom, top, min_bin_width, min_bin_height, min_derivative, identity_init, KB);
    a.lds_per_wave = ((128 * ST + 3) / 4) * 4;
    static_assert(128 * ST >= 32 * 128, "the chunk buffer holds the z1 tile");
    const size_t shmem = sizeof(float) * (size_t)FW * a.lds_per_wave;
    const int64_t n_wg = ((B + 31) / 32 + FW - 1) / FW;
    BGK_CHECK_ARG(n_wg < (int64_t)0x7fffffff, "%s: batch too large for one launch", what);
    hipStream_t st = (hipStream_t)stream;
#define BGK_LAUNCH(A, F) do { (void)hipFuncSetAttribute(reinterpret_cast<const void*>(coupling_rqs_bwd_recompute_kernel<A, F>), hipFuncAttributeMaxDynamicSharedMemorySize, 160 * 1024); \
                              hipLaunchKernelGGL((coupling_rqs_bwd_recompute_kernel<A, F>), dim3((int)n_wg), dim3(FTHREADS), shmem, st, a); } while (0)
#define BGK_LAUNCH_F(A) do { if (bgk_rc_vjp_variant == 1) BGK_LAUNCH(A, false); else BGK_LAUNCH(A, true); } while (0)
    if (act == 1) BGK_LAUNCH_F(1); else if (act == 2) BGK_LAUNCH_F(2); else BGK_LAUNCH_F(3);
#undef BGK_LAUNCH_F
#undef BGK_LAUNCH
    return bgk_launch_status(what);
}
#endif

#if !BGK_V2_AFFTRAIN
#if BGK_V2_SAVE
int bgk_launch_rqs_dense_h2v2_train(const char* what, float* z0, float* z1, float* params, int64_t ldp, const int32_t* src_col,
                                    const float* cond, int64_t ldc, int32_t d_c, int32_t periodic,
#elif BGK_V2_BF16
int bgk_launch_rqs_dense_h2v2_bf16(const char* what, const float* cond, int64_t ldc, int32_t d_c, int32_t periodic,
#else
int bgk_launch_rqs_dense_h2v2(const char* what, const float* cond, int64_t ldc, int32_t d_c, int32_t periodic,
#endif
                              const void* A0p, const void* A1p, const void* A2p, float c0, float c1, float c2, const float* cs_dev,
                              int32_t act, const float* y, int64_t ldy, int64_t B, int32_t d, uint64_t circ_mask, int32_t inverse,
                              double left, double right, double bottom, double top,
                              double min_bin_width, double min_bin_height, double min_derivative, int32_t identity_init,
                              float* out, int64_t ldo, float* dlogp, int32_t accumulate, int32_t* bin_idx, int32_t* oob_count,
                              void* stream, const BgkCondSegs* segs) {
    V2Args a;
    const int n_in = periodic ? 2 * d_c : d_c;
    BGK_CHECK_ARG(make_cond_segs(a.cs, cond, ldc, d_c, segs), "%s: bad conditioning segments", what);
    a.d_c = d_c; a.periodic = periodic;
    a.y = y; a.ldy = ldy; a.out = out; a.ldo = ldo; a.d = d; a.magic_d = magic_div(d);
    a.B = B; a.dlogp = dlogp; a.accumulate = accumulate; a.bin_idx = bin_idx; a.oob_count = oob_count;
    a.A0 = reinterpret_cast<const uint4*>(A0p); a.A1 = reinterpret_cast<const uint4*>(A1p); a.A2 = reinterpret_cast<const uint4*>(A2p);
    a.S0 = (n_in + 1 + 15) / 16;
    a.n_chunks = (d + DPC - 1) / DPC;
    a.last_tiles = ((d - (a.n_chunks - 1) * DPC) * PPD + 31) / 32;
    a.c0 = c0; a.c1 = c1; a.c2 = c2; a.cs_dev = cs_dev;
    a.circ_mask = circ_mask;
    a.sc.left = (float)left; a.sc.right = (float)right;
    const SetK sw = make_set(left, right, min_bin_width, KB), sh = make_set(bottom, top, min_bin_height, KB);
    a.sc.sa = inverse ? sw : sh;
    a.sc.sb = inverse ? sh : sw;
    const double beta = identity_init ? (0.6931471805599453 / (1.0 - min_derivative)) : 1.0;
    a.sc.beta = (float)beta; a.sc.kout = (float)(0.6931471805599453 / (double)(float)beta); a.sc.min_d = (float)min_derivative;
    const TilePlan tp = plan_tiles(a.cs, d_c, periodic, y, ldy, out, ldo, d, 128 * ST);
    a.nfs = tp.nfs; a.ys = tp.ys; a.stage = tp.stage; a.y_dma = tp.y_dma; a.out_lin = tp.out_lin;
    BGK_CHECK_ARG(32 * a.nfs + 16 <= 128 * ST, "%s: %d conditioner input features do not fit the LDS tile", what, n_in);
    a.lds_per_wave = ((128 * ST + 32 * a.ys + 32 + 3) / 4) * 4;
#if BGK_V2_SAVE
    a.z0 = z0; a.z1 = z1; a.params = params; a.ldp = ldp; a.src_col = src_col;
#endif
    const size_t shmem = sizeof(float) * (size_t)FW * a.lds_per_wave;
    const int64_t n_wg = ((B + 31) / 32 + FW - 1) / FW;
    BGK_CHECK_ARG(n_wg < (int64_t)0x7fffffff, "%s: batch too large for one launch", what);
    BGK_CHECK_ARG((int64_t)32 * (d > d_c ? d : d_c) < (1 << 16), "%s: tile index range", what);
    BGK_CHECK_ARG(ldy < (1 << 24) && ldo < (1 << 24), "%s: row stride too large", what);
    const int grid = (int)n_wg;
    hipStream_t st = (hipStream_t)stream;
#if BGK_V2_SAVE
#define BGK_LAUNCH(A, I) do { if (params) hipLaunchKernelGGL((coupling_rqs_dense_h2v2_kernel<A, I, true>), dim3(grid), dim3(FTHREADS), shmem, st, a); \
                              else hipLaunchKernelGGL((coupling_rqs_dense_h2v2_kernel<A, I, false>), dim3(grid), dim3(FTHREADS), shmem, st, a); } while (0)
#else
#define BGK_LAUNCH(A, I) hipLaunchKernelGGL((coupling_rqs_dense_h2v2_kernel<A, I>), dim3(grid), dim3(FTHREADS), shmem, st, a)
#endif
    if (act == 1) { if (inverse) BGK_LAUNCH(1, 1); else BGK_LAUNCH(1, 0); }
    else if (act == 2) { if (inverse) BGK_LAUNCH(2, 1); else BGK_LAUNCH(2, 0); }
    else { if (inverse) BGK_LAUNCH(3, 1); else BGK_LAUNCH(3, 0); }
#undef BGK_LAUNCH
    return bgk_launch_status(what);
}
#endif

#if !BGK_V2_SAVE && !BGK_V2_BF16
#if BGK_V2_AFFTRAIN
int bgk_launch_affine_dense_v2_train(const BgkAffTrainSave* save,
                               const float* cond, int64_t ldc, int32_t d_c, int32_t periodic,
#else
int bgk_launch_affine_dense_v2(const float* cond, int64_t ldc, int32_t d_c, int32_t periodic,
#endif
                               const void* sA0, const void* sA1, const void* sA1b, const void* sA2, float sc0, float sc1, float sc1b, float sc2, int32_t s_act,
                               const void* tA0, const void* tA1, const void* tA1b, const void* tA2, float tc0, float tc1, float tc1b, float tc2, int32_t t_act,
                               const float* log_alpha, int32_t preserve_volume, int32_t is_circular, int32_t inverse,
                               const float* y, int64_t ldy, int64_t B, int32_t d,
                               float* out, int64_t ldo, float* dlogp, int32_t accumulate, void* stream, const BgkCondSegs* segs) {
#if BGK_V2_AFFTRAIN
    const char* what = "bgk_coupling_affine_dense_h2_train";
#else
    const char* what = "bgk_coupling_affine_dense_h2";
#endif
    AffV2Args a;
    const int n_in = periodic ? 2 * d_c : d_c;
    BGK_CHECK_ARG(make_cond_segs(a.cs, cond, ldc, d_c, segs), "%s: bad conditioning segments", what);
    a.d_c = d_c; a.periodic = periodic; a.S0 = (n_in + 1 + 15) / 16;
#if BGK_V2_AFFTRAIN
    a.shift = AffV2Net{(const uint4*)sA0, (const uint4*)sA1, (const uint4*)sA1b, (const uint4*)sA2, sc0, sc1, sc1b, sc2, save->s_cs, save->s_z0, save->s_z1};
    a.scale = AffV2Net{(const uint4*)tA0, (const uint4*)tA1, (const uint4*)tA1b, (const uint4*)tA2, tc0, tc1, tc1b, tc2, save->t_cs, save->t_z0, save->t_z1};
    a.mu_out = save->mu; a.s_out = save->s_raw; a.ldms = save->ldms; a.zt = save->ldz == 64 ? 2 : 4;
#else
    a.shift = AffV2Net{(const uint4*)sA0, (const uint4*)sA1, (const uint4*)sA1b, (const uint4*)sA2, sc0, sc1, sc1b, sc2};
    a.scale = AffV2Net{(const uint4*)tA0, (const uint4*)tA1, (const uint4*)tA1b, (const uint4*)tA2, tc0, tc1, tc1b, tc2};
#endif
    a.has_shift = sA0 != nullptr; a.has_scale = tA0 != nullptr;
    const bool deep = a.has_shift ? sA1b != nullptr : tA1b != nullptr;
#if BGK_V2_AFFTRAIN
    if (deep) return BGK_EUNSUPPORTED;
    BGK_CHECK_ARG((!a.has_shift || (save->s_z0 && save->s_z1 && save->mu)) && (!a.has_scale || (save->t_z0 && save->t_z1 && save->s_raw)),
                  "%s: null save buffer", what);
    BGK_CHECK_ARG(save->ldz == 64 || save->ldz == 128, "%s: ldz = %lld (64 | 128)", what, (long long)save->ldz);
    BGK_CHECK_ARG(save->ldms >= 32 * ((d + 31) / 32) && save->ldms % 4 == 0 && save->ldms < (1 << 20), "%s: ldms = %lld (a multiple of 4, >= 32 ceil(d / 32))",
                  what, (long long)save->ldms);
#endif
    if (a.has_shift && a.has_scale && (sA1b != nullptr) != (tA1b != nullptr)) return BGK_EUNSUPPORTED;
    const int as = a.has_shift ? s_act : t_act, at = a.has_scale ? t_act : s_act;
    if (!((as == at && as >= 1 && as <= 3) || (as == 2 && at == 3))) return BGK_EUNSUPPORTED;
    a.log_alpha = log_alpha; a.preserve_volume = preserve_volume; a.is_circular = is_circular; a.inverse = inverse;
    a.y = y; a.ldy = ldy; a.B = B; a.d = d; a.out = out; a.ldo = ldo; a.dlogp = dlogp; a.accumulate = accumulate;
    a.magic_d = magic_div(d);
    const int OT = (d + 31) / 32;
    TilePlan tp = plan_tiles(a.cs, d_c, periodic, y, ldy, out, ldo, d, 32 * 128);
    a.nfs = tp.nfs; a.ys = tp.ys; a.stage = tp.stage; a.y_dma = tp.y_dma; a.out_lin = tp.out_lin;
    const int tile_f = 32 * a.nfs + (a.stage == 2 ? 32 * d_c : 0) + 16, park_f = d * SROW;
    a.lds_tile = (((tile_f > park_f ? tile_f : park_f) + 3) / 4) * 4;
#if BGK_V2_AFFTRAIN
    a.slab = a.lds_tile;
    a.lds_tile += 16 * 32;
#endif
    a.lds_per_wave = a.lds_tile + ((32 * a.ys + 3) / 4) * 4;
    const size_t shmem = sizeof(float) * (size_t)FW * a.lds_per_wave;
    const int64_t n_wg = ((B + 31) / 32 + FW - 1) / FW;
    BGK_CHECK_ARG(n_wg < (int64_t)0x7fffffff, "%s: batch too large for one launch", what);
    BGK_CHECK_ARG(ldy < (1 << 24) && ldo < (1 << 24) && (int64_t)32 * d_c < 4096 && (int64_t)32 * d < 4096
                  && OT >= 1 && OT <= 3, "%s: outside the kernel's envelope", what);
    if (shmem > 160 * 1024) {
        bgk_set_error("%s: %d input features / %d dims do not fit the LDS tiles", what, n_in, d);
        return BGK_EUNSUPPORTED;
    }
    hipStream_t st = (hipStream_t)stream;
#define BGK_LAUNCH(S, T, O, D) do { if (shmem > 64 * 1024) (void)hipFuncSetAttribute(reinterpret_cast<const void*>(coupling_affine_dense_v2_kernel<S, T, O, D>), \
                                        hipFuncAttributeMaxDynamicSharedMemorySize, 160 * 1024); \
                                    hipLaunchKernelGGL((coupling_affine_dense_v2_kernel<S, T, O, D>), dim3((int)n_wg), dim3(FTHREADS), shmem, st, a); } while (0)
#if BGK_V2_AFFTRAIN
#define BGK_LAUNCH_D(S, T, O) BGK_LAUNCH(S, T, O, false)
#else
#define BGK_LAUNCH_D(S, T, O) do { if (deep) BGK_LAUNCH(S, T, O, true); else BGK_LAUNCH(S, T, O, false); } while (0)
#endif
#define BGK_LAUNCH_O(S, T) do { if (OT == 1) BGK_LAUNCH_D(S, T, 1); else if (OT == 2) BGK_LAUNCH_D(S, T, 2); else BGK_LAUNCH_D(S, T, 3); } while (0)
    if (as == 1) BGK_LAUNCH_O(1, 1); else if (as == 3) BGK_LAUNCH_O(3, 3); else if (at == 2) BGK_LAUNCH_O(2, 2); else BGK_LAUNCH_O(2, 3);
#undef BGK_LAUNCH_D
#undef BGK_LAUNCH_O
#undef BGK_LAUNCH
    return bgk_launch_status(what);
}
#endif
```

bgflow_amd/dense.py:

```python
import ctypes
import os
import weakref

import numpy as np
import torch

from . import _lib
from .utils import is_list_or_tuple, param_pitch, param_state_key, row_pitch

__all__ = ["DenseNet", "MeanFreeDenseNet", "WrapPeriodic", "WrapDistances"]


def _matmul_nn(g, w):
    return torch.nn.functional.linear(g, w.t().contiguous())


def _gram_tn(g, h, splits=64):
    B = g.shape[0]
    if B % splits or B // splits < 256:
        return g.t() @ h
    return torch.bmm(g.view(splits, B // splits, -1).transpose(1, 2), h.view(splits, B // splits, -1)).sum(0)


def column_sum(g, nblk=1024):
# ... 892 lines not shown
                and all(lin.out_features <= 128 for lin in deep[0][:-1]):
            return _deep_plan(transformer, net, deep, periodic, y_dim, nc_slot_host)
        if type(inner) is DenseNet:
            return _reject(transformer, "the fused spline kernels take a DenseNet with biases and one of SiLU / ReLU / Tanh: two hidden "
                                        "layers of up to 256 units, or (mode 'f16x2') 1 .. 8 hidden layers of up to 128")
        return None
    (l0, l1, l2), act = spec
    H_max = max(l0.out_features, l1.out_features)
    if H_max > 256:
        return _reject(transformer, f"hidden layers ({l0.out_features}, {l1.out_features}): widths up to 256 are fused")
    if H_max > 128 and mode != "f16x2":
        return _reject(transformer, f"hidden layers ({l0.out_features}, {l1.out_features}) in gemm_mode '{mode}': widths above 128 are "
                                    f"fused in mode 'f16x2' only")
    H_run = 128 if H_max <= 128 else 256
    padded = (l0.out_features, l1.out_features) != (H_run, H_run)
    if y_dim > 64:
        return _reject(transformer, f"{y_dim} transformed dims: at most 64 are fused")
    n_nc = int((nc_slot_host >= 0).sum())
    P = l2.out_features
    n_bins = (P - n_nc) // (3 * y_dim)
    if 3 * n_bins * y_dim + n_nc != P:
        return None
    if n_bins != 8 and not (n_bins in (4, 12, 16, 32) and mode == "f16x2"):
        return _reject(transformer, f"{n_bins} bins in gemm_mode '{mode}': fused for 8 bins, and for 4 / 12 / 16 / 32 bins in mode 'f16x2'"
                                    + ("; more than 64 bins run on device torch ops" if n_bins > 64 else ""))
    d_c = l0.in_features // 2 if periodic else l0.in_features
    if periodic:
        idx = np.arange(d_c)[net.indices] if not isinstance(net.indices, slice) or net.indices != slice(None) else np.arange(d_c)
        if len(idx) != d_c or 2 * d_c != l0.in_features or not np.array_equal(np.asarray(idx), np.arange(d_c)):
            return _reject(transformer, "WrapPeriodic over a subset / permutation of the conditioner inputs")
    params = [p for lin in (l0, l1, l2) for p in (lin.weight, lin.bias)]
    version = tuple(param_state_key(p) for p in params)
    cache = transformer._fused_cache
    dev = l0.weight.device
    stale = cache.get("version") != version
    if cache.get("y_dim") != y_dim or cache.get("mode") != mode or cache.get("device") != dev:
        cache.clear()
        stale = True
    if stale:
        common = dict(version=version, y_dim=y_dim, mode=mode, device=dev, act=act, periodic=periodic, d_c=d_c, n_bins=n_bins,
                      padded=padded, hidden=H_run, circ_mask=int(sum(1 << j for j in range(y_dim) if nc_slot_host[j] < 0)))
        if padded:
            l0, l1, l2 = _pad_hidden((l0, l1, l2), H_run)
        if mode == "bf16" and dev.type != "cuda":
            return None
        if H_run == 256:
            cache.update(common, packed=pack_dense_for_fused_w256((l0, l1, l2), nc_slot_host, y_dim, n_bins), cs=None)
            cache.pop("bufs", None)
        elif mode == "bf16" or (mode == "f16x2" and dev.type == "cuda"):
            if "src_col_dev" not in cache:
                cache["src_col_dev"] = _src_col_table(y_dim, n_bins, nc_slot_host, dev)
            n_chunks = cache["src_col_dev"].numel() // 128
            A0, A1, A2, cs = pack_dense_for_fused_h2_device((l0, l1, l2), cache["src_col_dev"], n_chunks, cache.get("bufs"),
                                                            bf16=(mode == "bf16"))
            cache.update(common, bufs=(A0, A1, A2, cs), packed=(A0, A1, A2, (1.0, 1.0, 1.0)), cs=cs)
        else:
            pack = pack_dense_for_fused if mode == "f32" else pack_dense_for_fused_h2
            cache.update(common, packed=pack((l0, l1, l2), nc_slot_host, y_dim, n_bins), cs=None)
            cache.pop("bufs", None)
    return cache


def _deep_plan(transformer, net, spec, periodic, y_dim, nc_slot_host):
    lins, act = spec
    if y_dim > 64:
        return _reject(transformer, f"{y_dim} transformed dims: at most 64 are fused")
    n_nc = int((nc_slot_host >= 0).sum())
    P = lins[-1].out_features
    n_bins = (P - n_nc) // (3 * y_dim)
    if 3 * n_bins * y_dim + n_nc != P:
        return None
    if n_bins not in (4, 8, 12, 16, 32):
        return _reject(transformer, f"{n_bins} bins: the one-launch kernels take 4 / 8 / 12 / 16 / 32")
    l0 = lins[0]
    d_c = l0.in_features // 2 if periodic else l0.in_features
    if periodic:
        idx = np.arange(d_c)[net.indices] if not isinstance(net.indices, slice) or net.indices != slice(None) else np.arange(d_c)
        if len(idx) != d_c or 2 * d_c != l0.in_features or not np.array_equal(np.asarray(idx), np.arange(d_c)):
            return _reject(transformer, "WrapPeriodic over a subset / permutation of the conditioner inputs")
    version = tuple(param_state_key(p) for lin in lins for p in (lin.weight, lin.bias))
    cache = transformer._fused_cache
    dev = l0.weight.device
    if cache.get("version") != version or cache.get("y_dim") != y_dim or cache.get("mode") != "f16x2" or cache.get("device") != dev \
            or not cache.get("deep"):
        cache.clear()
        padded = any(lin.out_features != 128 for lin in lins[:-1])
        run = _pad_hidden(lins, 128) if padded else lins
        cache.update(version=version, y_dim=y_dim, mode="f16x2", device=dev, act=act, periodic=periodic, d_c=d_c, n_bins=n_bins,
                     padded=padded, hidden=128, deep=len(lins) - 1, cs=None,
                     circ_mask=int(sum(1 << j for j in range(y_dim) if nc_slot_host[j] < 0)),
                     packed=pack_dense_for_fused_deep(run, nc_slot_host, y_dim, n_bins))
    return cache


def fused_spline_coupling(transformer, x, y, nc_slot_host, inverse, oob_counter, want_bin_idx=False, acc=None):
    if x.dim() != 2 or y.dim() != 2 or not x.is_cuda:
        return None
    plan = _fused_plan(transformer, y.shape[-1], nc_slot_host)
    if plan is None or x.shape[-1] != plan["d_c"]:
        return None
    parts = _cond_parts(x)
    if len(parts) > 1 and (plan["mode"] == "f32" or plan["n_bins"] != 8 or plan["hidden"] != 128 or plan.get("deep")):
        parts = [x.cat()]
    _lib.require_hip(y, *parts)
    W0p, W1p, W2p = plan["packed"][:3]
    if W0p.device != y.device:
        return None
    y2, ldy = _lib.rowmajor(y)
    B, d = y2.shape
    out = torch.empty((B, d), dtype=torch.float32, device=y.device)
    if acc is not None:
        dlogp, accumulate = acc.peek()
    else:
        dlogp, accumulate = torch.empty((B,), dtype=torch.float32, device=y.device), False
    bins = torch.empty((B, d), dtype=torch.int32, device=y.device) if want_bin_idx else None
    s = transformer._default_settings
    tail = (plan["hidden"], plan["hidden"], plan["act"], _lib.ptr(y2), ldy, B, d, plan["n_bins"], plan["circ_mask"], int(inverse),
            transformer._left, transformer._right, transformer._bottom, transformer._top,
            s["min_bin_width"], s["min_bin_height"], s["min_derivative"], int(s.get("enable_identity_init", False)),
            _lib.ptr(out), d, _lib.ptr(dlogp), int(bool(accumulate)), _lib.ptr(bins), _lib.ptr(oob_counter), _lib.stream_ptr(y.device))
    with torch.cuda.device(y.device):
        if plan.get("deep"):
            A0, A1, A2, c0, c1s, c2 = plan["packed"]
            x2, ldc = _lib.rowmajor(parts[0])
            c1_arr = (ctypes.c_float * max(1, len(c1s)))(*c1s)
            st = _lib.lib().bgk_coupling_rqs_dense_deep(
                _lib.ptr(x2), ldc, plan["d_c"], int(plan["periodic"]), _lib.ptr(A0), _lib.ptr(A1), _lib.ptr(A2), c0, c1_arr, c2,
                plan["deep"], *tail[2:])
        elif plan["mode"] == "f32":
            x2, ldc = _lib.rowmajor(parts[0])
            st = _lib.lib().bgk_coupling_rqs_dense(
                _lib.ptr(x2), ldc, plan["d_c"], int(plan["periodic"]), _lib.ptr(W0p), _lib.ptr(W1p), _lib.ptr(W2p), *tail)
        else:
            c0, c1, c2 = plan["packed"][3]
            ops = (_lib.ptr(W0p), _lib.ptr(W1p), _lib.ptr(W2p), c0, c1, c2, _lib.ptr(plan.get("cs")), int(plan["mode"] == "bf16"))
            st = -2
            if len(parts) > 1:
                ptrs, lds, widths, n, keep = _lib.cond_segments(parts)
                st = _lib.lib().bgk_coupling_rqs_dense_h2_mc(ptrs, lds, widths, n, int(plan["periodic"]), *ops, *tail)
                if st == -2:
                    parts = [x.cat()]
            if st == -2:
                x2, ldc = _lib.rowmajor(parts[0])
                st = _lib.lib().bgk_coupling_rqs_dense_h2(_lib.ptr(x2), ldc, plan["d_c"], int(plan["periodic"]), *ops, *tail)
    if st == -2:
        return _reject(transformer, "shape outside the fused spline kernels' envelope: " + _lib.lib().bgk_last_error().decode(errors="replace"))
    _lib.check(st, "bgk_coupling_rqs_dense")
    if acc is not None:
        acc.commit()
    res = (out, acc if acc is not None else dlogp[:, None])
    return res + (bins,) if want_bin_idx else res


def _act_fwd_bwd(code):
    if code == 1:
        return torch.nn.functional.silu, lambda g, z, h: torch.ops.aten.silu_backward(g, z)
    if code == 2:
        return torch.relu, lambda g, z, h: g * (z > 0).to(g.dtype)
    return torch.tanh, lambda g, z, h: g * (1.0 - h * h)


def _featurise(x, periodic):
    if not periodic:
        return x
    ang = 2 * np.pi * x
    return torch.cat([torch.cos(ang), torch.sin(ang)], dim=-1)


PACKED_PARAMS = True
RECOMPUTE_PARAMS = True


def absmax_of(*tensors):
    dev = next(t for t in tensors if t is not None).device
    out = torch.zeros(len(tensors), dtype=torch.float32, device=dev)
    with torch.cuda.device(dev):
        for i, t in enumerate(tensors):
            if t is None or t.numel() == 0:
                continue
            t2, ld = _lib.rowmajor(t.detach())
            _lib.check(_lib.lib().bgk_absmax(_lib.ptr(t2), ld, t2.shape[0], t2.shape[1], _lib.ptr(out[i:]), _lib.stream_ptr(dev)), "bgk_absmax")
    return out


def _dense_backward_dx(g_p, z1, z0, x, W0, W1, W2, cs, act_code, periodic, want_gx, bufs, want_h=True, t_version=None, absmax=None,
                       gx_add=None, gx_out=None):
    dev = g_p.device
    B, P = g_p.shape
    n_in = W0.shape[1]
    _t_operand_bufs(bufs, P, n_in, dev)
    T0, T1, T2 = bufs["T0"], bufs["T1"], bufs["T2"]
    g2, ldg = _lib.rowmajor(g_p)
    x2, ldc = _lib.rowmajor(x.detach())
    d_c = x2.shape[1]
    n_out = 4 if want_h else 2
    out = torch.empty((n_out, B, 128), dtype=torch.float32, device=dev)
    g_x = (gx_out if gx_out is not None else torch.empty((B, d_c), dtype=torch.float32, device=dev)) if want_gx else None
    add2, lda = _lib.rowmajor(gx_add) if (gx_add is not None and want_gx) else (None, 0)
    ws = [w.detach().contiguous() for w in (W0, W1, W2)]
    with torch.cuda.device(dev):
        if t_version is None or bufs.get("t_version") != t_version:
            st = _lib.lib().bgk_pack_dense_h2_t(_lib.ptr(ws[0]), n_in, _lib.ptr(ws[1]), _lib.ptr(ws[2]), P, _lib.ptr(cs),
                                                _lib.ptr(T0), _lib.ptr(T1), _lib.ptr(T2), _lib.stream_ptr(dev))
            _lib.check(st, "bgk_pack_dense_h2_t")
            bufs["t_version"] = t_version
        st = _lib.lib().bgk_dense_backward_dx(_lib.ptr(g2), ldg, P, _lib.ptr(z1), _lib.ptr(z0), _lib.ptr(x2), ldc, d_c, int(periodic),
                                              _lib.ptr(T0), _lib.ptr(T1), _lib.ptr(T2), _lib.ptr(cs), act_code, B,
                                              _lib.ptr(out[0]), _lib.ptr(out[1]), _lib.ptr(out[2]) if want_h else None,
                                              _lib.ptr(out[3]) if want_h else None, _lib.ptr(g_x), _lib.rowmajor(g_x)[1] if g_x is not None else d_c,
                                              _lib.ptr(add2), lda, _lib.ptr(absmax), _lib.ptr(absmax[1:]) if absmax is not None else None, _lib.stream_ptr(dev))
        _lib.check(st, "bgk_dense_backward_dx")
    return out[0], out[1], (out[2] if want_h else None), (out[3] if want_h else None), g_x


_DIRECT_GRADS = [False]


DEFERRED_WGRAD_REDUCE = True

_PENDING_REDUCE = {}


def flush_weight_grad_reductions():
    if not _PENDING_REDUCE:
        return
    by_dev = {}
    for dev, *rest in _PENDING_REDUCE.values():
        by_dev.setdefault(dev, []).append(rest)
    _PENDING_REDUCE.clear()
    for dev, items in by_dev.items():
        n = len(items)
        vps, i32s = ctypes.c_void_p * n, ctypes.c_int32 * n
        dst = lambda k: vps(*[it[4][k].data_ptr() for it in items])
        with torch.cuda.device(dev):
            st = _lib.lib().bgk_mlp_weight_grad_reduce_many(
                n, (ctypes.c_int64 * n)(*[it[0] for it in items]), i32s(*[it[1] for it in items]),
                i32s(*[it[5] for it in items]), i32s(*[it[6] for it in items]),
                i32s(*[it[2] for it in items]), vps(*[it[3].data_ptr() for it in items]),
                dst(4), dst(5), dst(2), dst(3), dst(0), dst(1), 1, _lib.stream_ptr(dev))
        _lib.check(st, "bgk_mlp_weight_grad_reduce_many")


class direct_grad_accumulation:

    def __enter__(self):
        self._prev = _DIRECT_GRADS[0]
        _DIRECT_GRADS[0] = True
        return self

    def __exit__(self, *exc):
        _DIRECT_GRADS[0] = self._prev
        if not self._prev:
            if exc[0] is None:
                flush_weight_grad_reductions()
            else:
                _PENDING_REDUCE.clear()
        return False


def _dense_weight_grad(g_p, g_z1, g_z0, h1, h0, x, periodic, n_in, need, bufs, params=None, h_act=0, absmax=None):
    dev = g_p.device
    B, P = g_p.shape
    g2, ldg = _lib.rowmajor(g_p)
    x2, ldc = _lib.rowmajor(x)
    lib = _lib.lib()
    need_ws = int(lib.bgk_dense_weight_grad_workspace(B, P, n_in))
    ws = bufs.get("wgrad_ws")
    if ws is None or ws.numel() < need_ws or ws.device != dev:
        ws = bufs["wgrad_ws"] = torch.empty(need_ws, dtype=torch.float32, device=dev)
    direct = _DIRECT_GRADS[0] and params is not None and all(need[2:8]) and all(
        getattr(p, "_bgk_grad_dst", None) is not None and p.grad is not None and p.grad.data_ptr() == p._bgk_grad_dst.data_ptr()
        for p in params)
    if direct:
        gW0, gb0, gW1, gb1, gW2, gb2 = (p._bgk_grad_dst for p in params)
    else:
        gW2 = torch.empty((P, 128), dtype=torch.float32, device=dev) if need[6] else None
        gb2 = torch.empty((P,), dtype=torch.float32, device=dev) if need[7] else None
        gW1 = torch.empty((128, 128), dtype=torch.float32, device=dev) if need[4] else None
        gb1 = torch.empty((128,), dtype=torch.float32, device=dev) if need[5] else None
        gW0 = torch.empty((128, n_in), dtype=torch.float32, device=dev) if need[2] else None
        gb0 = torch.empty((128,), dtype=torch.float32, device=dev) if need[3] else None

    def wbuf(w, b, shape):
        return w if (w is not None or b is None) else torch.empty(shape, dtype=torch.float32, device=dev)
    w2, w1, w0 = wbuf(gW2, gb2, (P, 128)), wbuf(gW1, gb1, (128, 128)), wbuf(gW0, gb0, (128, n_in))
    if absmax is None:
        absmax = absmax_of(g_p, g_z1, g_z0)
    mode = int(direct)
    if direct and DEFERRED_WGRAD_REDUCE:
        if ws.data_ptr() in _PENDING_REDUCE:
            flush_weight_grad_reductions()
        _PENDING_REDUCE[ws.data_ptr()] = (dev, B, P, n_in, ws, (gW0, gb0, gW1, gb1, gW2, gb2), 128, 128)
        mode = 2
    with torch.cuda.device(dev):
        st = lib.bgk_dense_weight_grad(_lib.ptr(g2), ldg, P, _lib.ptr(g_z1), _lib.ptr(g_z0), _lib.ptr(h1), _lib.ptr(h0), int(h_act),
                                       _lib.ptr(x2), ldc, x2.shape[1], int(periodic), B, _lib.ptr(ws), ws.numel(),
                                       _lib.ptr(w2), _lib.ptr(gb2), _lib.ptr(w1), _lib.ptr(gb1), _lib.ptr(w0), _lib.ptr(gb0),
                                       mode, _lib.ptr(absmax), _lib.stream_ptr(dev))
    _lib.check(st, "bgk_dense_weight_grad")
    if direct:
        return (None,) * 6
    return gW0, gb0, gW1, gb1, gW2, gb2


def _train_forward_launch(x, y, W2, plan, tcfg, inverse, oob, dlogp=None, accumulate=False):
    A0, A1, A2, (c0, c1, c2) = plan["packed"]
# ... 784 lines not shown
```

bgflow_amd/flow.py:

```python
import warnings
from collections.abc import Sequence

import numpy as np
import torch

__all__ = [
    "Flow", "SequentialFlow", "InverseFlow", "SplitFlow", "MergeFlow", "SwapFlow", "CouplingFlow",
    "WrapFlow", "SetConstantFlow", "StochasticAugmentation",
]


class Flow(torch.nn.Module):

    def _forward(self, *xs, **kwargs):
        raise NotImplementedError()

    def _inverse(self, *xs, **kwargs):
        raise NotImplementedError()

    def forward(self, *xs, inverse=False, **kwargs):
        return self._inverse(*xs, **kwargs) if inverse else self._forward(*xs, **kwargs)


def _zero_dlogp(x):
    return torch.zeros(*x.shape[:-1], 1, dtype=x.dtype, device=x.device)


ACC_KW = "_bgk_logdet"


class _LogDetAcc:
    __slots__ = ("buf", "started")

    def __init__(self, batch, device):
        self.buf = torch.empty(batch, dtype=torch.float32, device=device)
        self.started = False

    def target(self):
        acc = self.started
        self.started = True
        return self.buf, acc

    def peek(self):
        return self.buf, self.started

    def commit(self):
        self.started = True

    def add(self, t):
        if t is self or t is None:
            return
        t = t.reshape(-1) if torch.is_tensor(t) else t
        if self.started:
            self.buf.add_(t)
        elif torch.is_tensor(t):
            self.buf.copy_(t)
            self.started = True
        else:
            self.buf.fill_(float(t))
            self.started = True

    def result(self):
        if not self.started:
            self.buf.zero_()
            self.started = True
        return self.buf[:, None]


class CatView:
    __slots__ = ("parts", "_cat")

    def __init__(self, parts):
        self.parts = tuple(parts)
        self._cat = None

    @property
    def shape(self):
        return torch.Size([self.parts[0].shape[0], sum(t.shape[1] for t in self.parts)])

    device = property(lambda self: self.parts[0].device)
    dtype = property(lambda self: self.parts[0].dtype)
    is_cuda = property(lambda self: self.parts[0].is_cuda)
    requires_grad = False

    def dim(self):
        return 2

    def cat(self):
        if self._cat is None:
            self._cat = torch.cat(self.parts, dim=-1)
        return self._cat


def as_tensor(x):
    return x.cat() if isinstance(x, CatView) else x


def _acc_kwargs(flow, kwargs):
    if ACC_KW in kwargs and not getattr(flow, "_bgk_acc", False):
        kwargs = {k: v for k, v in kwargs.items() if k != ACC_KW}
    return kwargs


def _acc_eligible(xs):
    x = xs[0] if xs else None
    if not (torch.is_tensor(x) and x.is_cuda and x.dtype == torch.float32 and x.dim() == 2):
        return False
    if torch.is_grad_enabled() and any(torch.is_tensor(t) and t.requires_grad for t in xs):
        return False
    return True


class SequentialFlow(Flow):

    def __init__(self, blocks):
        super().__init__()
        self._blocks = torch.nn.ModuleList(blocks)

    FUSE_GENERATION_TAIL = True
    FUSE_TRAINING_TAIL = True
    FUSE_COUPLING_STACKS = True
    FUSE_TRAINING_CHAINS = True
    FUSE_CONSTANT_MERGE = True

    _bgk_acc = True
    ACCUMULATE_IN_KERNELS = True

    def forward(self, *xs, inverse=False, **kwargs):
        return self.run(xs, inverse=inverse, kwargs=kwargs)

    FUSE_KL_EPILOGUE = True

    def kl_sums(self, xs, target, temperature=1.0, drop_nonfinite=False):
        from .distributions import _kernel_plan
        if not (self.FUSE_KL_EPILOGUE and torch.is_grad_enabled() and isinstance(temperature, (int, float)) and temperature > 0):
            return None
        segs = self.segments(inverse=False, train=True)
        tail = segs[-1][1] if segs else None
        if not isinstance(tail, _FusedGenerationTail):
            return None
        plan = _kernel_plan(target, temperature)
        if plan is None:
            return None
        specs, dims, c_in, c_out, t_eff = plan
        ic = tail._ic
        n_cart = 3 * (getattr(ic, "_rel_ic", ic)._n + getattr(ic, "_rel_ic", ic)._n_fixed)
        if not (len(specs) == 1 and specs[0][0] == 0 and dims == [n_cart]):
            return None
        total = None
        for _label, seg in segs[:-1]:
            *xs, dd = seg(*xs, inverse=False, temperature=temperature)
            total = dd if total is None else total + dd
        if len(xs) != 4:
            res = None
        else:
            res = tail.kl_sums(tuple(xs), total, (specs, t_eff, c_in, c_out), drop_nonfinite)
        if res is not None:
            return res
        from .distributions import kl_loss_sums
        *x, dd = tail(*xs, inverse=False, temperature=temperature)
        total = dd if total is None else total + dd
        out = kl_loss_sums(target, tuple(x), total, temperature=temperature, drop_nonfinite=drop_nonfinite)
        if out is not None:
            return out[0]
        per = target.energy(*x, temperature=temperature) - total
        if drop_nonfinite:
            ok = torch.isfinite(per)
            return torch.stack([torch.where(ok, per, torch.zeros_like(per)).sum().to(torch.float64), ok.sum().to(torch.float64)])
        return torch.stack([per.sum().to(torch.float64), torch.tensor(float(per.numel()), dtype=torch.float64, device=per.device)])

    def run(self, xs, inverse=False, kwargs=None, around=None):
        kwargs = dict(kwargs or {})
        outer = kwargs.pop(ACC_KW, None)
        acc = outer
        if acc is None and self.ACCUMULATE_IN_KERNELS and _acc_eligible(xs) and not (
                torch.is_grad_enabled() and any(p.requires_grad for p in self.parameters())):
            acc = _LogDetAcc(xs[0].shape[0], xs[0].device)
        if acc is None:
            total = None
            for i, (label, seg) in enumerate(self.segments(inverse=inverse, train=True)):
                if around is None:
                    *xs, ddlogp = seg(*xs, inverse=inverse, **kwargs)
                else:
                    with around(i, label):
                        *xs, ddlogp = seg(*xs, inverse=inverse, **kwargs)
                total = ddlogp if total is None else total + ddlogp
            return (*xs, 0.0 if total is None else total)
        kwargs[ACC_KW] = acc
        for i, (label, seg) in enumerate(self.segments(inverse=inverse)):
            kw = _acc_kwargs(seg, kwargs)
            if around is None:
                *xs, ddlogp = seg(*xs, inverse=inverse, **kw)
                acc.add(ddlogp)
            else:
                with around(i, label):
                    *xs, ddlogp = seg(*xs, inverse=inverse, **kw)
                    acc.add(ddlogp)
        return (*xs, acc if outer is not None else acc.result())

    def segments(self, inverse=False, train=False):
        blocks = list(self._blocks)
        train = bool(train) and self.FUSE_TRAINING_CHAINS
        key = (self.FUSE_GENERATION_TAIL, self.FUSE_COUPLING_STACKS, self.FUSE_CONSTANT_MERGE, tuple(id(b) for b in blocks))
        cache = self.__dict__.setdefault("_segment_cache", {})
        if cache.get("key") != key:
            cache.clear()
            cache["key"] = key
        which = (bool(inverse), train)
        if which not in cache:
            segs = self._build_segments(blocks, inverse)
            cache[which] = _with_train_chains(segs) if train else segs
        return cache[which]

    def _build_segments(self, blocks, inverse):
        tail = self._generation_tail() if self.FUSE_GENERATION_TAIL else None
        if inverse:
            if tail is None:
                return self._with_coupling_stacks(list(reversed(blocks)), True)
            return [("xyz2ic+cdf", _FusedInferenceHead(self, tail))] + self._with_coupling_stacks(list(reversed(blocks[:tail[0]])), True)
        if tail is None:
            return self._with_coupling_stacks(blocks, False)
        start = tail[0]
        return self._with_coupling_stacks(blocks[:start], False) + [("icdf+ic2xyz", _FusedGenerationTail(self, tail))]

    def _with_coupling_stacks(self, blocks, inverse):
        from .modulo import FusedConstantMerge, constant_merge_pair
        out, i = [], 0
        while i < len(blocks):
            pair = constant_merge_pair(blocks[i], blocks[i + 1], inverse) if self.FUSE_CONSTANT_MERGE and i + 1 < len(blocks) else None
            if pair is not None:
                out.append(("constant merge", FusedConstantMerge(*pair)))
                i += 2
                continue
            j = _coupling_stack_end(blocks, i, inverse) if self.FUSE_COUPLING_STACKS else None
            if j is None:
                out.append((type(blocks[i]).__name__, blocks[i]))
                i += 1
            else:
                out.append(("coupling stack", _FusedCouplingStack(blocks[i:j + 1])))
                i = j + 1
        return out

    def _generation_tail(self):
        from .cdf import CDFTransform
        blocks = list(self._blocks)
        if len(blocks) < 2:
            return None
        last = blocks[-1]
        ic = getattr(getattr(last, "_flow", None), "_delegate", None)
        if not (type(last) is WrapFlow and type(last._flow) is InverseFlow and hasattr(ic, "_generate_fused")
                and list(last._indices) == [0, 1, 2, 3] and list(last._out_indices) == [0]):
            return None
        maps, others = {}, []
        i = len(blocks) - 1
        while i - 1 >= 0:
            b = blocks[i - 1]
            cdf = getattr(getattr(b, "_flow", None), "_delegate", None)
            if not (type(b) is WrapFlow and type(b._flow) is InverseFlow and type(cdf) is CDFTransform and len(b._indices) == 1
                    and list(b._out_indices) == list(b._indices) and b._indices[0] not in maps):
                break
            if b._indices[0] in (0, 1, 2, 3):
                maps[b._indices[0]] = cdf
            else:
                others.insert(0, b)
            i -= 1
        if not maps:
            return None
        eps = {c._eps for c in maps.values()}
        if len(eps) != 1:
            return None
        return i, maps, ic, eps.pop(), others

    def _forward(self, *args, **kwargs):
        return self.forward(*args, **kwargs, inverse=False)

    def _inverse(self, *args, **kwargs):
        return self.forward(*args, **kwargs, inverse=True)

    def trigger(self, function_name):
        results = [getattr(b, function_name)() for b in self._blocks
                   if callable(getattr(b, function_name, None))]
        if results and all(r is not None for r in results):
            return torch.stack(results)
        return torch.zeros(0)

    def __iter__(self):
        return iter(self._blocks)

    def __len__(self):
        return len(self._blocks)

    def __getitem__(self, index):
        if isinstance(index, int):
            return self._blocks[index]
        picked = np.arange(len(self))[index]
        return SequentialFlow([self._blocks[i] for i in picked])


def _with_train_chains(segs):
    from .transformer import ConditionalSplineTransformer
    out, run = [], []

    def flush():
        if len(run) >= 2:
            out.append(("spline chain", _SplineTrainChain([b for _, b in run])))
        else:
            out.extend(run)
        run.clear()
    for label, seg in segs:
        if type(seg) is CouplingFlow and type(seg.transformer) is ConditionalSplineTransformer and seg.cat_dim == -1 \
                and len(seg.transformed_indices) == 1 and len(seg.cond_indices) == 1:
            run.append((label, seg))
        else:
            flush()
            out.append((label, seg))
    flush()
    return out


class _SplineTrainChain:

    _bgk_acc = True

    def __init__(self, blocks):
        self._blocks = blocks

    def _blocks_path(self, *xs, inverse=False, **kwargs):
        acc = kwargs.get(ACC_KW)
        total = None
        for block in self._blocks:
            *xs, dd = block(*xs, inverse=inverse, **_acc_kwargs(block, kwargs))
            if acc is not None:
                acc.add(dd)
            else:
                total = dd if total is None else total + dd
        return (*xs, acc if acc is not None else total)

    def __call__(self, *xs, inverse=False, **kwargs):
        from .dense import spline_chain_train
        if kwargs.get(ACC_KW) is None and not set(kwargs) - {"temperature"} and torch.is_grad_enabled() and (
                any(torch.is_tensor(x) and x.requires_grad for x in xs)
                or any(p.requires_grad for b in self._blocks for p in b.parameters())):
            res = spline_chain_train(self._blocks, xs, inverse)
            if res is not None:
                return (*res[0], res[1])
        return self._blocks_path(*xs, inverse=inverse, **kwargs)


def _split_sizes(block, inverse, merging):
    split = block if type(block) is SplitFlow else (block._delegate if type(block) is MergeFlow else None)
    if split is None or split._indices is not None or split._split_dim != -1 or len(split._sizes) not in (1, 2):
        return None
    acts_as_merge = (type(block) is MergeFlow) != bool(inverse)
    return tuple(split._sizes) if acts_as_merge == merging else None


def _coupling_stack_end(blocks, i, inverse):
    from .transformer import AffineTransformer
    sizes = _split_sizes(blocks[i], inverse, merging=False)
    if sizes is None:
        return None
    n_couplings, swapped = 0, False
    for j in range(i + 1, len(blocks)):
        b = blocks[j]
        if type(b) is SwapFlow:
            swapped = not swapped
            continue
        if type(b) is CouplingFlow and type(b.transformer) is AffineTransformer and tuple(b.transformed_indices) == (1,) \
                and tuple(b.cond_indices) == (0,) and b.cat_dim == -1:
            n_couplings += 1
            continue
        closing = _split_sizes(b, inverse, merging=True)
        if closing is None or n_couplings < 2:
            return None
        if swapped:
            return j if (len(sizes) < 2 or closing[0] == sizes[1]) else None
        return j if closing[0] == sizes[0] else None
    return None


class _FusedCouplingStack:

    _bgk_acc = True
    FUSE_TRAINING_STACK = True

    def __init__(self, blocks):
        self._blocks = blocks

    def _blocks_path(self, *xs, inverse=False, **kwargs):
        acc = kwargs.get(ACC_KW)
        total = 0.0
        for block in self._blocks:
            *xs, dd = block(*xs, inverse=inverse, **_acc_kwargs(block, kwargs))
            if acc is not None:
                acc.add(dd)
            else:
                total = total + dd
        return (*xs, acc if acc is not None else total)

    def __call__(self, *xs, inverse=False, **kwargs):
        from .dense import fused_affine_coupling, _affine_plan, _gemm_mode
        acc = kwargs.get(ACC_KW)
        kwargs_rest = {k: v for k, v in kwargs.items() if k != ACC_KW}
        x = xs[0] if len(xs) == 1 else None
        ok = (x is not None and not set(kwargs_rest) - {"temperature"} and torch.is_tensor(x) and x.is_cuda and x.dtype == torch.float32
              and x.dim() == 2 and x.is_contiguous() and x.shape[0] > 0)
        couplings = [b for b in self._blocks if type(b) is CouplingFlow]
        if ok and torch.is_grad_enabled() and (x.requires_grad or any(p.requires_grad for b in couplings for p in b.parameters())):
            ok = False
            if acc is None and self.FUSE_TRAINING_STACK:
                from .dense import affine_stack_train
                res = affine_stack_train(self._blocks, x, inverse)
                if res is not None:
                    return res
        if ok:
            split = self._blocks[0] if type(self._blocks[0]) is SplitFlow else self._blocks[0]._delegate
            s0, D = split._sizes[0], x.shape[1]
            ok = 0 < s0 < D and (len(split._sizes) == 1 or split._sizes[1] == D - s0)
        if ok:
            widths = (s0, D - s0)
            part = [0, 1]
            for b in self._blocks[1:-1]:
                if type(b) is SwapFlow:
                    part.reverse()
                    continue
                tr = b.transformer
                if not getattr(tr, "allow_fused", False) or _gemm_mode(tr) == "f32" or _affine_plan(tr, widths[part[1]]) is None \
                        or tr._fused_cache.get("d_c") != widths[part[0]]:
                    ok = False
                    break
            if ok:
                closing = self._blocks[-1] if type(self._blocks[-1]) is SplitFlow else self._blocks[-1]._delegate
                ok = closing._sizes[0] == widths[part[0]] and (len(closing._sizes) == 1 or closing._sizes[1] == widths[part[1]])
        if not ok:
            return self._blocks_path(*xs, inverse=inverse, **kwargs)
        B = x.shape[0]
        work = torch.empty_like(x)
        if acc is not None:
            dlogp, started = acc.target()
        else:
            dlogp, started = torch.empty(B, dtype=torch.float32, device=x.device), False
        cols = (slice(0, s0), slice(s0, D))
        where = [x, x]
        part, first = [0, 1], not started
        for b in self._blocks[1:-1]:
            if type(b) is SwapFlow:
                part.reverse()
                continue
            pc, py = part
# ... 489 lines not shown
```

include/bgflow_amd.h:

```cpp
#ifndef BGFLOW_AMD_H
#define BGFLOW_AMD_H

#include <stdint.h>

#ifdef __cplusplus
extern "C" {
#endif

#pragma GCC visibility push(default)

#define BGK_EINVAL (-1)
#define BGK_EUNSUPPORTED (-2)

int bgk_abi_version(void);
const char* bgk_last_error(void);

int bgk_set_option(int32_t option, int32_t value);

int bgk_detmath_probe(const float* x, int64_t n, int32_t which, float* out, void* stream);

int bgk_rqs_transform(const float* y, int64_t ldy, const float* params, int64_t ldp, int32_t P,
                      const int32_t* nc_slot, int64_t B, int32_t d, int32_t K, int32_t inverse,
                      double left, double right, double bottom, double top,
                      double min_bin_width, double min_bin_height, double min_derivative,
                      int32_t identity_init,
                      float* out, int64_t ldo, float* dlogp, int32_t accumulate,
                      int32_t* bin_idx, int32_t* oob_count, void* stream);

int bgk_rqs_backward(const float* y, int64_t ldy, const float* params, int64_t ldp, int32_t P,
                     const int32_t* nc_slot, int64_t B, int32_t d, int32_t K, int32_t inverse,
                     double left, double right, double bottom, double top,
                     double min_bin_width, double min_bin_height, double min_derivative,
                     int32_t identity_init,
                     const float* g_out, int64_t ldgo, const float* g_dlogp,
                     float* g_y, int64_t ldgy, float* g_params, int64_t ldgp, float* g_absmax, int32_t params_layout, void* stream);

int bgk_affine_transform(const float* y, int64_t ldy, const float* mu, int64_t ldmu,
                         const float* s_raw, int64_t lds, const float* log_alpha,
                         int32_t preserve_volume, int32_t is_circular, int32_t inverse,
                         int64_t B, int32_t d, float* out, int64_t ldo,
                         float* dlogp, int32_t accumulate, void* stream);

int bgk_affine_backward(const float* y, int64_t ldy, const float* mu, int64_t ldmu,
                        const float* s_raw, int64_t lds, const float* log_alpha,
                        int32_t preserve_volume, int32_t is_circular, int32_t inverse,
                        int64_t B, int32_t d,
                        const float* g_out, int64_t ldgo, const float* g_dlogp,
                        float* g_y, int64_t ldgy, float* g_mu, int64_t ldgmu,
                        float* g_s, int64_t ldgs, float* g_log_alpha, float* g_mu_absmax, float* g_s_absmax, void* stream);

int bgk_ic_xyz2ic(const float* x, int64_t ldx, const int32_t* zmat, int32_t n,
                  const int32_t* fixed, int32_t n_fixed, int32_t normalize_angles, float eps,
                  int32_t enforce_boundaries,
                  const float* wh_mean, const float* Twhiten, int32_t keep, float jac_xz,
                  int64_t B, float* bonds, float* angles, float* torsions, int64_t ldic,
                  float* xfix, int64_t ldf, float* dlogp, int32_t accumulate,
                  int32_t* warn_count, void* stream);

int bgk_ic_ic2xyz(const float* bonds, const float* angles, const float* torsions, int64_t ldic,
                  const float* xfix, int64_t ldf, const int32_t* place, int32_t n,
                  const int32_t* fixed, int32_t n_fixed, int32_t normalize_angles, float eps,
                  int32_t enforce_boundaries,
                  const float* wh_mean, const float* Tblacken, int32_t keep, float jac_xz,
                  int64_t B, float* x, int64_t ldx, float* dlogp, int32_t accumulate,
                  int32_t* warn_count, void* stream);

int bgk_ic_refsys(const float* in, int64_t B, int32_t inverse, int32_t normalize_angles, float eps,
                  int32_t enforce_boundaries, float* out, float* dlogp, int32_t accumulate, void* stream);

int bgk_icdf_ic2xyz(const float* bonds, const float* angles, const float* torsions, int64_t ldic,
                    const float* xfix, int64_t ldf,
                    const float* desc_bonds, const float* desc_angles, const float* desc_torsions, const float* desc_fixed,
                    int32_t use_eps, float cdf_eps,
                    const int32_t* place, int32_t n, const int32_t* fixed, int32_t n_fixed,
                    int32_t normalize_angles, float eps, int32_t enforce_boundaries,
                    const float* wh_mean, const float* Tblacken, int32_t keep, float jac_xz, int64_t B,
                    float* x, int64_t ldx, float* dlogp, int32_t accumulate, int32_t* warn_count, void* stream);

int bgk_icdf_ic2xyz_reg(const float* bonds, const float* angles, const float* torsions, const float* xfix,
                        const float* desc20, int32_t use_eps, float cdf_eps,
                        const int32_t* place8, int32_t n, const int32_t* fixed, int32_t n_fixed,
                        float eps, int32_t enforce_boundaries,
                        const float* wh_mean, const float* Tblacken, int32_t keep, double const_ld, int64_t B,
                        float* x, int64_t ldx, float* dlogp, int32_t accumulate, int32_t* warn_count, void* stream);

int bgk_icdf_ic2xyz_uni(const float* bonds, const float* angles, const float* torsions, const float* xfix,
                        const float* desc4, int32_t use_eps, float cdf_eps,
                        const int32_t* place8, int32_t n, const int32_t* fixed, int32_t n_fixed,
                        float eps, int32_t enforce_boundaries,
                        const float* wh_mean, const float* Tblacken, int32_t keep, double const_ld, int64_t B,
                        float* x, int64_t ldx, float* dlogp, int32_t accumulate, int32_t* warn_count, void* stream);
int bgk_icdf_ic2xyz_uni_train(const float* bonds, const float* angles, const float* torsions, const float* xfix,
                              const float* desc4, int32_t use_eps, float cdf_eps,
                              const int32_t* place8, int32_t n, const int32_t* fixed, int32_t n_fixed,
                              float eps, int32_t enforce_boundaries,
                              const float* wh_mean, const float* Tblacken, int32_t keep, double const_ld, int64_t B,
                              float* x, int64_t ldx, float* dlogp, int32_t accumulate, int32_t* warn_count,
                              float* y_bonds, float* y_angles, float* y_torsions, float* y_fixed, void* stream);
int bgk_icdf_ic2xyz_uni_train_kl(const float* bonds, const float* angles, const float* torsions, const float* xfix,
                                 const float* desc4, int32_t use_eps, float cdf_eps,
                                 const int32_t* place8, int32_t n, const int32_t* fixed, int32_t n_fixed,
                                 float eps, int32_t enforce_boundaries,
                                 const float* wh_mean, const float* Tblacken, int32_t keep, double const_ld, int64_t B,
                                 float* x, int64_t ldx, const float* dlogp_in, int32_t* warn_count,
                                 float* y_bonds, float* y_angles, float* y_torsions, float* y_fixed,
                                 const float* t_mean, double temperature, double c_in, double c_out, int32_t drop_nonfinite,
                                 float* u, float* dlogp_total, float* partial, double* loss_sums, void* stream);

int bgk_xyz2ic_cdf_uni(const float* x, const float* desc4, int32_t use_eps, float cdf_eps,
                       const int32_t* zmat8, int32_t n, const int32_t* fixed, int32_t n_fixed,
                       float eps, int32_t enforce_boundaries,
                       const float* wh_mean, const float* Twhiten, int32_t keep, double const_ld, int64_t B,
                       float* bonds, float* angles, float* torsions, float* xfix,
                       float* dlogp, int32_t accumulate, int32_t* warn_count, void* stream);

int bgk_ic_ic2xyz_backward(const float* bonds, const float* angles, const float* torsions, int64_t ldic,
                           const float* x, int64_t ldx, const int32_t* place, int32_t n,
                           const int32_t* fixed, int32_t n_fixed, int32_t normalize_angles,
                           float eps, int32_t enforce_boundaries,
                           const float* Tblacken, int32_t keep, int64_t B,
                           const float* g_x, int64_t ldgx, const float* g_dlogp,
                           float* g_bonds, float* g_angles, float* g_torsions, int64_t ldgic,
                           float* g_xfix, int64_t ldgf, int32_t* fix_ws, void* stream);

int bgk_ic_xyz2ic_backward(const float* x, int64_t ldx, const int32_t* zmat, int32_t n,
                           const int32_t* fixed, int32_t n_fixed, int32_t normalize_angles, float eps,
                           int32_t enforce_boundaries, const float* Twhiten, int32_t keep, int64_t B,
                           const float* g_bonds, const float* g_angles, const float* g_torsions, int64_t ldgic,
                           const float* g_xfix, int64_t ldgf, const float* g_dlogp,
                           float* g_x, int64_t ldgx, void* stream);

int bgk_ic_refsys_backward(const float* in, const float* g_out, const float* g_dlogp, int64_t B, int32_t inverse,
                           int32_t normalize_angles, float eps, int32_t enforce_boundaries, float* g_in, void* stream);

int bgk_cdf_transform(const float* x, int64_t ldx, const float* desc, int64_t B, int32_t d,
                      int32_t inverse, int32_t use_eps, float eps, float* out, int64_t ldo,
                      float* dlogp, int32_t accumulate, void* stream);

int bgk_cdf_backward(const float* x, int64_t ldx, const float* y, int64_t ldy, const float* desc, int64_t B, int32_t d,
                     int32_t inverse, int32_t use_eps, float eps, const float* g_y, int64_t ldgy,
                     const float* g_dlogp, float* g_x, int64_t ldgx, void* stream);

int bgk_coupling_rqs_dense(const float* cond, int64_t ldc, int32_t d_c, int32_t periodic,
                           const float* W0p, const float* W1p, const float* W2p,
                           int32_t H0, int32_t H1, int32_t act,
                           const float* y, int64_t ldy, int64_t B, int32_t d, int32_t K,
                           uint64_t circ_mask, int32_t inverse,
                           double left, double right, double bottom, double top,
                           double min_bin_width, double min_bin_height, double min_derivative,
                           int32_t identity_init,
                           float* out, int64_t ldo, float* dlogp, int32_t accumulate,
                           int32_t* bin_idx, int32_t* oob_count, void* stream);

int bgk_coupling_rqs_dense_h2(const float* cond, int64_t ldc, int32_t d_c, int32_t periodic,
                              const void* A0p, const void* A1p, const void* A2p,
                              float c0, float c1, float c2, const float* cs_dev, int32_t operand_dtype,
                              int32_t H0, int32_t H1, int32_t act,
                              const float* y, int64_t ldy, int64_t B, int32_t d, int32_t K,
                              uint64_t circ_mask, int32_t inverse,
                              double left, double right, double bottom, double top,
                              double min_bin_width, double min_bin_height, double min_derivative,
                              int32_t identity_init,
                              float* out, int64_t ldo, float* dlogp, int32_t accumulate,
                              int32_t* bin_idx, int32_t* oob_count, void* stream);

int bgk_coupling_rqs_dense_deep(const float* cond, int64_t ldc, int32_t d_c, int32_t periodic,
                                const void* A0p, const void* A1p, const void* A2p, float c0, const float* c1s, float c2,
                                int32_t n_hidden, int32_t act,
                                const float* y, int64_t ldy, int64_t B, int32_t d, int32_t K,
                                uint64_t circ_mask, int32_t inverse,
                                double left, double right, double bottom, double top,
                                double min_bin_width, double min_bin_height, double min_derivative,
                                int32_t identity_init,
                                float* out, int64_t ldo, float* dlogp, int32_t accumulate,
                                int32_t* bin_idx, int32_t* oob_count, void* stream);

int bgk_coupling_rqs_dense_h2_train(const float* cond, int64_t ldc, int32_t d_c, int32_t periodic,
                                    const void* A0p, const void* A1p, const void* A2p,
                                    float c0, float c1, float c2, const float* cs_dev,
                                    int32_t H0, int32_t H1, int32_t act,
                                    const float* y, int64_t ldy, int64_t B, int32_t d, int32_t K,
                                    uint64_t circ_mask, int32_t inverse,
                                    double left, double right, double bottom, double top,
                                    double min_bin_width, double min_bin_height, double min_derivative,
                                    int32_t identity_init,
                                    float* out, int64_t ldo, float* dlogp, int32_t accumulate,
                                    int32_t* oob_count, float* z0, float* z1, float* params, int64_t ldp,
                                    const int32_t* src_col_dev, int32_t params_layout, void* stream);
int bgk_coupling_rqs_dense_h2_backward(const float* z1, const void* A2p, float c2, const float* cs_dev, int32_t H1, int32_t act,
                                       const float* y, int64_t ldy, int64_t B, int32_t d, int32_t K, int32_t P,
                                       uint64_t circ_mask, int32_t inverse,
                                       double left, double right, double bottom, double top,
                                       double min_bin_width, double min_bin_height, double min_derivative,
                                       int32_t identity_init, const float* g_out, int64_t ldgo, const float* g_dlogp,
                                       float* g_y, int64_t ldgy, float* g_params, int64_t ldgp, float* g_absmax, void* stream);

int bgk_coupling_affine_dense_h2(const float* cond, int64_t ldc, int32_t d_c, int32_t periodic,
                                 const void* sA0, const void* sA1, const void* sA2,
                                 float sc0, float sc1, float sc2, int32_t s_act,
                                 const void* tA0, const void* tA1, const void* tA2,
                                 float tc0, float tc1, float tc2, int32_t t_act,
                                 int32_t hidden, const float* log_alpha, int32_t preserve_volume,
                                 int32_t is_circular, int32_t inverse,
                                 const float* y, int64_t ldy, int64_t B, int32_t d,
                                 float* out, int64_t ldo, float* dlogp, int32_t accumulate, void* stream);

int bgk_coupling_affine_dense_h3(const float* cond, int64_t ldc, int32_t d_c, int32_t periodic,
                                 const void* sA0, const void* sA1, const void* sA1b, const void* sA2,
                                 float sc0, float sc1, float sc1b, float sc2, int32_t s_act,
                                 const void* tA0, const void* tA1, const void* tA1b, const void* tA2,
                                 float tc0, float tc1, float tc1b, float tc2, int32_t t_act,
                                 int32_t hidden, const float* log_alpha, int32_t preserve_volume,
                                 int32_t is_circular, int32_t inverse,
                                 const float* y, int64_t ldy, int64_t B, int32_t d,
                                 float* out, int64_t ldo, float* dlogp, int32_t accumulate, void* stream);

int bgk_coupling_affine_dense_deep(const float* cond, int64_t ldc, int32_t d_c, int32_t periodic,
                                   const void* sA0, const void* sA1, const void* sA2, float sc0, const float* sc1s, float sc2, int32_t s_act,
                                   const void* tA0, const void* tA1, const void* tA2, float tc0, const float* tc1s, float tc2, int32_t t_act,
                                   int32_t n_hidden, int32_t hidden, const float* log_alpha, int32_t preserve_volume,
                                   int32_t is_circular, int32_t inverse,
                                   const float* y, int64_t ldy, int64_t B, int32_t d,
                                   float* out, int64_t ldo, float* dlogp, int32_t accumulate, void* stream);

int bgk_coupling_affine_dense_h2_train(const float* const* cond, const int64_t* ldc, const int32_t* width, int32_t n_cond, int32_t periodic,
                                       const void* sA0, const void* sA1, const void* sA2, const float* s_cs, int32_t s_act,
                                       const void* tA0, const void* tA1, const void* tA2, const float* t_cs, int32_t t_act,
                                       const float* log_alpha, int32_t preserve_volume, int32_t is_circular, int32_t inverse,
                                       const float* y, int64_t ldy, int64_t B, int32_t d, float* out, int64_t ldo,
                                       float* dlogp, int32_t accumulate,
                                       float* s_z0, float* s_z1, float* t_z0, float* t_z1, int64_t ldz,
                                       float* mu, float* s_raw, int64_t ldms, void* stream);

int bgk_coupling_rqs_dense_h2_mc(const float* const* cond, const int64_t* ldc, const int32_t* width, int32_t n_cond, int32_t periodic,
                                 const void* A0p, const void* A1p, const void* A2p,
                                 float c0, float c1, float c2, const float* cs_dev, int32_t operand_dtype,
                                 int32_t H0, int32_t H1, int32_t act,
                                 const float* y, int64_t ldy, int64_t B, int32_t d, int32_t K,
                                 uint64_t circ_mask, int32_t inverse,
                                 double left, double right, double bottom, double top,
                                 double min_bin_width, double min_bin_height, double min_derivative,
                                 int32_t identity_init,
                                 float* out, int64_t ldo, float* dlogp, int32_t accumulate,
                                 int32_t* bin_idx, int32_t* oob_count, void* stream);
int bgk_coupling_affine_dense_h2_mc(const float* const* cond, const int64_t* ldc, const int32_t* width, int32_t n_cond, int32_t periodic,
                                    const void* sA0, const void* sA1, const void* sA2,
                                    float sc0, float sc1, float sc2, int32_t s_act,
                                    const void* tA0, const void* tA1, const void* tA2,
                                    float tc0, float tc1, float tc2, int32_t t_act,
                                    int32_t hidden, const float* log_alpha, int32_t preserve_volume,
                                    int32_t is_circular, int32_t inverse,
                                    const float* y, int64_t ldy, int64_t B, int32_t d,
                                    float* out, int64_t ldo, float* dlogp, int32_t accumulate, void* stream);
int bgk_coupling_affine_dense_h3_mc(const float* const* cond, const int64_t* ldc, const int32_t* width, int32_t n_cond, int32_t periodic,
                                    const void* sA0, const void* sA1, const void* sA1b, const void* sA2,
                                    float sc0, float sc1, float sc1b, float sc2, int32_t s_act,
                                    const void* tA0, const void* tA1, const void* tA1b, const void* tA2,
                                    float tc0, float tc1, float tc1b, float tc2, int32_t t_act,
                                    int32_t hidden, const float* log_alpha, int32_t preserve_volume,
                                    int32_t is_circular, int32_t inverse,
                                    const float* y, int64_t ldy, int64_t B, int32_t d,
                                    float* out, int64_t ldo, float* dlogp, int32_t accumulate, void* stream);

int bgk_pack_dense_h2(const float* W0, const float* b0, int32_t n_in, int32_t H,
                      const float* W1, const float* b1,
                      const float* W2, const float* b2, int32_t rows2,
                      const int32_t* row_map2_dev, int32_t n_groups2, int32_t NT2, int32_t operand_dtype,
                      void* A0, void* A1, void* A2, float* cs, void* stream);

int bgk_pack_dense_h2_many(int32_t n, const float* const* W0, const float* const* b0, const int32_t* n_in,
                           const float* const* W1, const float* const* b1, const float* const* W2, const float* const* b2,
                           const int32_t* rows2, const int32_t* const* row_map2_dev, const int32_t* n_groups2,
                           void* const* A0, void* const* A1, void* const* A2, float* const* cs, void* stream);

int bgk_pack_mlp_h2(const float* W0, const float* b0, int32_t n_in, int32_t H0,
                    const float* W1, const float* b1, int32_t H1,
                    const float* W2, const float* b2, int32_t rows2,
                    const int32_t* row_map2_dev, int32_t n_groups2, int32_t NT2, int32_t HT,
                    void* A0, void* A1, void* A2, float* cs, void* stream);
int bgk_pack_mlp_h2_many(int32_t n, const float* const* W0, const float* const* b0, const int32_t* n_in, const int32_t* H0,
                         const float* const* W1, const float* const* b1, const int32_t* H1,
                         const float* const* W2, const float* const* b2,
                         const int32_t* rows2, const int32_t* const* row_map2_dev, const int32_t* n_groups2, const int32_t* NT2,
                         const int32_t* HT,
                         void* const* A0, void* const* A1, void* const* A2, float* const* cs, void* stream);

int bgk_pack_dense_h2_t(const float* W0, int32_t n_in, const float* W1, const float* W2, int32_t P,
                        const float* cs, void* T0, void* T1, void* T2, void* stream);
int bgk_pack_mlp_h2_t(const float* W0, int32_t n_in, int32_t H0, const float* W1, int32_t H1, const float* W2, int32_t P,
                      const float* cs, void* T0, void* T1, void* T2, void* stream);
int bgk_pack_mlp_h2_t_many(int32_t n, const float* const* W0, const int32_t* n_in, const int32_t* H0, const float* const* W1,
                           const int32_t* H1, const float* const* W2, const int32_t* P, const float* const* cs,
                           void* const* T0, void* const* T1, void* const* T2, void* stream);

int bgk_pack_dense_h2_t_many(int32_t n, const float* const* W0, const int32_t* n_in, const float* const* W1,
                             const float* const* W2, const int32_t* P, const float* const* cs,
                             void* const* T0, void* const* T1, void* const* T2, void* stream);
int bgk_mlp_backward_dx(const float* g, int64_t ldg, int32_t P, const float* z1, const float* z0, int64_t ldz,
                        const float* cond, int64_t ldc, int32_t d_c, int32_t periodic,
                        const void* T0, const void* T1, const void* T2, const float* cs, int32_t act,
                        int64_t B, float* g_z1, float* g_z0, float* h1, float* h0,
                        float* g_cond, int64_t ldgc, const float* g_cond_add, int64_t ldga,
                        const float* g_absmax, float* gz_absmax, void* stream);
int bgk_dense_backward_dx(const float* g, int64_t ldg, int32_t P, const float* z1, const float* z0,
                          const float* cond, int64_t ldc, int32_t d_c, int32_t periodic,
                          const void* T0, const void* T1, const void* T2, const float* cs, int32_t act,
                          int64_t B, float* g_z1, float* g_z0, float* h1, float* h0,
                          float* g_cond, int64_t ldgc, const float* g_cond_add, int64_t ldga,
                          const float* g_absmax, float* gz_absmax, void* stream);

int bgk_grad_nan_flag(const float* g, int64_t n, int32_t* flag, void* stream);
int bgk_adam_step(float* p, const float* g, float* m, float* v, int64_t n, float lr, float beta1, float beta2, float eps,
                  float weight_decay, int64_t step, const int32_t* skip_flag, int32_t* skipped_count, void* stream);

int bgk_normal_energy(const float* x, int64_t ldx, const float* mean, int32_t d, int64_t B,
                      double temperature, double log_z, float* u, void* stream);
int bgk_normal_energy_backward(const float* x, int64_t ldx, const float* mean, int32_t d, int64_t B,
// ... 109 lines not shown
```

Before: 133.2 million.

## Fuse consecutive spline coupling layers into one persistent chain kernel for inference

Adds a chain kernel that keeps both feature halves of a 32-row tile resident in LDS and runs several consecutive RQS coupling layers (conditioner MLP plus spline) in one launch. Per-layer parameters come from a device-side table that is built once and cached. The flow driver now detects runs of compatible coupling segments and dispatches them to this path, falling back to the per-layer path otherwise. This is meant to remove the global-memory round trips and launch overhead between layers, at the cost of a more complex kernel, possible register and LDS pressure, and a new table-caching path.

```diff
diff --git a/bgflow_amd/_lib.py b/bgflow_amd/_lib.py
--- a/bgflow_amd/_lib.py
+++ b/bgflow_amd/_lib.py
@@ -72,6 +72,11 @@
                                                  vp, i64, i64, i32, i32, ctypes.c_uint64, i32,
                                                  f64, f64, f64, f64, f64, f64, f64, i32,
                                                  vp, i64, vp, i32, vp, vp, vp]),
+    "bgk_coupling_rqs_chain_layer_size": (ctypes.c_int64, []),
+    "bgk_coupling_rqs_chain_layer": (ctypes.c_int, [vp, i32, i32, i32, i32, i32, vp, vp, vp, f32, f32, f32, vp,
+                                                    i32, i32, i32, ctypes.c_uint64, i32,
+                                                    f64, f64, f64, f64, f64, f64, f64, i32, vp]),
+    "bgk_coupling_rqs_dense_h2_chain": (ctypes.c_int, [vp, i32, i32, i32, vp, vp, i32, i32, vp, vp, i64, vp, i32, vp]),
     "bgk_coupling_rqs_dense_deep": (ctypes.c_int, [vp, i64, i32, i32, vp, vp, vp, f32, vp, f32, i32, i32,
                                                    vp, i64, i64, i32, i32, ctypes.c_uint64, i32,
                                                    f64, f64, f64, f64, f64, f64, f64, i32,
diff --git a/bgflow_amd/csrc/bgk_capi.hip b/bgflow_amd/csrc/bgk_capi.hip
--- a/bgflow_amd/csrc/bgk_capi.hip
+++ b/bgflow_amd/csrc/bgk_capi.hip
@@ -37,6 +37,28 @@
     return BGK_EINVAL;
 }
 
+extern "C" int64_t bgk_coupling_rqs_chain_layer_size(void) { return bgk_rqs_chain_layer_size(); }
+
+extern "C" int bgk_coupling_rqs_chain_layer(void* table_host, int32_t index, int32_t transformed, int32_t w0, int32_t w1, int32_t periodic,
+                                            const void* A0p, const void* A1p, const void* A2p,
+                                            float c0, float c1, float c2, const float* cs_dev,
+                                            int32_t H0, int32_t H1, int32_t K, uint64_t circ_mask, int32_t inverse,
+                                            double left, double right, double bottom, double top,
+                                            double min_bin_width, double min_bin_height, double min_derivative,
+                                            int32_t identity_init, int32_t* oob_count) {
+    return bgk_fill_rqs_chain_layer("bgk_coupling_rqs_chain_layer", table_host, index, transformed, w0, w1, periodic, A0p, A1p, A2p, c0, c1, c2,
+                                    cs_dev, H0, H1, K, circ_mask, inverse, left, right, bottom, top, min_bin_width, min_bin_height,
+                                    min_derivative, identity_init, oob_count);
+}
+
+extern "C" int bgk_coupling_rqs_dense_h2_chain(const void* table_dev, int32_t n_layers, int32_t act, int32_t inverse,
+                                               const float* in0, const float* in1, int32_t w0, int32_t w1,
+                                               float* out0, float* out1, int64_t B, float* dlogp, int32_t accumulate, void* stream) {
+    if (B == 0) return 0;
+    return bgk_launch_rqs_dense_h2v2_chain("bgk_coupling_rqs_dense_h2_chain", table_dev, n_layers, act, inverse, in0, in1, w0, w1, out0, out1, B,
+                                           dlogp, accumulate, stream);
+}
+
 namespace {
 __global__ void detmath_probe_kernel(const float* x, int64_t n, int which, float* out) {
     int64_t i = (int64_t)blockIdx.x * blockDim.x + threadIdx.x;
diff --git a/bgflow_amd/csrc/bgk_fused2.h b/bgflow_amd/csrc/bgk_fused2.h
--- a/bgflow_amd/csrc/bgk_fused2.h
+++ b/bgflow_amd/csrc/bgk_fused2.h
@@ -37,6 +37,16 @@
                                    float* out, int64_t ldo, float* dlogp, int32_t accumulate, int32_t* bin_idx, int32_t* oob_count,
                                    void* stream, const BgkCondSegs* segs = nullptr);
 
+int64_t bgk_rqs_chain_layer_size(void);
+int bgk_fill_rqs_chain_layer(const char* what, void* table_host, int32_t index, int32_t transformed, int32_t w0, int32_t w1, int32_t periodic,
+                             const void* A0p, const void* A1p, const void* A2p, float c0, float c1, float c2, const float* cs_dev,
+                             int32_t H0, int32_t H1, int32_t K, uint64_t circ_mask, int32_t inverse,
+                             double left, double right, double bottom, double top,
+                             double min_bin_width, double min_bin_height, double min_derivative, int32_t identity_init, int32_t* oob_count);
+int bgk_launch_rqs_dense_h2v2_chain(const char* what, const void* table_dev, int32_t n_layers, int32_t act, int32_t inverse,
+                                    const float* in0, const float* in1, int32_t w0, int32_t w1, float* out0, float* out1, int64_t B,
+                                    float* dlogp, int32_t accumulate, void* stream);
+
 int bgk_launch_affine_dense_v2(const float* cond, int64_t ldc, int32_t d_c, int32_t periodic,
                                const void* sA0, const void* sA1, const void* sA1b, const void* sA2, float sc0, float sc1, float sc1b, float sc2, int32_t s_act,
                                const void* tA0, const void* tA1, const void* tA1b, const void* tA2, float tc0, float tc1, float tc1b, float tc2, int32_t t_act,
diff --git a/bgflow_amd/csrc/bgk_fused2.hip b/bgflow_amd/csrc/bgk_fused2.hip
--- a/bgflow_amd/csrc/bgk_fused2.hip
+++ b/bgflow_amd/csrc/bgk_fused2.hip
@@ -1,3 +1,5 @@
+#include <string.h>
+
 #include "bgk_common.h"
 #include "bgk_fused2.h"
 
@@ -53,6 +55,9 @@
 #else
 #define V2_TS(k) do { } while (0)
 #endif
+#ifndef BGK_V2_ABL
+#define BGK_V2_ABL 0
+#endif
 constexpr int RD = BGK_V2_RD;
 constexpr int EH = 34;
 
@@ -70,6 +75,7 @@
 };
 
 struct V2Args {
+    static constexpr bool CLIP = false;
     CondSegs cs;
     int d_c; int periodic;
     const float* y; int64_t ldy; float* out; int64_t ldo; int d; uint32_t magic_d;
@@ -131,6 +137,9 @@
         rs = __builtin_amdgcn_make_buffer_rsrc((void*)W, 0, 0x7fffffff, 0x00020000);
         loads<0, RDX>();
         __builtin_amdgcn_sched_barrier(0);
+    }
+    __device__ __forceinline__ void attach() {
+        rs = __builtin_amdgcn_make_buffer_rsrc((void*)W, 0, 0x7fffffff, 0x00020000);
     }
     template <int E>
     __device__ __forceinline__ void event() {
@@ -270,10 +279,41 @@
     __device__ __forceinline__ const SpC& get() const { return a.sc; }
 };
 
-template <int INV, class H>
+typedef const __attribute__((address_space(4))) SpC* spc_t;
+struct CLArgs {
+    static constexpr bool CLIP = true;
+    const uint4* A2; uint64_t circ_mask; int ys, spare;
+    SpC sc; spc_t scp;
+};
+__device__ __forceinline__ void load_setk(SetK& o, const __attribute__((address_space(4))) SetK& s) {
+    o.gnum = s.gnum; o.low = s.low; o.high = s.high; o.dstep = s.dstep;
+#pragma unroll
+    for (int i = 0; i < 7; ++i) o.kc[i] = s.kc[i];
+}
+__device__ __forceinline__ void load_spc(SpC& o, spc_t p) {
+    o.left = p->left; o.right = p->right; o.beta = p->beta; o.kout = p->kout; o.min_d = p->min_d;
+    load_setk(o.sa, p->sa); load_setk(o.sb, p->sb);
+}
+template <bool KARG> struct ScSrcC;
+template <> struct ScSrcC<true> {
+    spc_t p;
+    __device__ __forceinline__ ScSrcC(const CLArgs& a) { p = a.scp; asm volatile("" : "+s"(p)); }
+    __device__ __forceinline__ const __attribute__((address_space(4))) SpC& get() const { return *p; }
+};
+template <> struct ScSrcC<false> {
+    const CLArgs& a;
+    __device__ __forceinline__ ScSrcC(const CLArgs& a_) : a(a_) {}
+    __device__ __forceinline__ const SpC& get() const { return a.sc; }
+};
+template <bool KARG, class AT> struct ScSel { typedef ScSrc<KARG> type; };
+template <bool KARG> struct ScSel<KARG, CLArgs> { typedef ScSrcC<KARG> type; };
+__device__ __forceinline__ int spare_off(const V2Args& a, int j) { return 32 * a.ys + j; }
+__device__ __forceinline__ int spare_off(const CLArgs& a, int j) { return a.spare + j; }
+
+template <int INV, class H, class AT>
 __device__ __forceinline__ float rqs_fast(H hk, float x, const float* pa, const float* pb, const float* ps, bool circ,
-                                          const V2Args& a, const SpK& k, float* lad, int* bin, int* oob) {
-    const ScSrc<(BGK_V2_KARG == 2 ? INV != 0 : BGK_V2_KARG != 0)> scs(a);
+                                          const AT& a, const SpK& k, float* lad, int* bin, int* oob) {
+    const typename ScSel<(BGK_V2_KARG == 2 ? INV != 0 : BGK_V2_KARG != 0), AT>::type scs(a);
 #define SC scs.get()
     float va[KB], vb[KB];
 #pragma unroll
@@ -453,8 +493,8 @@
 
 #undef SC
 
-template <int INV, int IT, int NHK, class G>
-__device__ __forceinline__ void spline_slot(G& g, const V2Args& a, const SpK& k, const float* s_p, float* s_y, int c, int nd,
+template <int INV, int IT, int NHK, class G, class AT>
+__device__ __forceinline__ void spline_slot(G& g, const AT& a, const SpK& k, const float* s_p, float* s_y, int c, int nd,
                                             int hh, int j, int rows, float& run, int& oob_local, int (&bins)[3]) {
     const int q = 2 * IT + hh;
     const bool valid = q < nd;
@@ -469,7 +509,7 @@
     const float x = s_y[j * a.ys + dim];
     Hooks<G, IT * EH, NHK> hk{g};
     const float o = rqs_fast<INV>(hk, x, INV ? pw : ph, INV ? ph : pw, ps, circ, a, k, &lad, &bin, &oob);
-    s_y[valid ? j * a.ys + dim : 32 * a.ys + j] = o;
+    s_y[valid ? j * a.ys + dim : spare_off(a, j)] = o;
     oob_local += (valid && j < rows) ? oob : 0;
     bins[IT] = bin;
     lad = valid ? lad : 0.0f;
@@ -479,11 +519,15 @@
     run += l1;
 }
 
+template <bool CLIP = false>
 __device__ __forceinline__ void chunk_to_lds(const f32x16 (&h)[4], float* s_p, int hh, int j) {
 #pragma unroll
     for (int m = 0; m < 4; ++m)
 #pragma unroll
-        for (int r = 0; r < 16; ++r) s_p[drow(m, r, hh) * ST + j] = h[m][r];
+        for (int r = 0; r < 16; ++r) {
+            if (CLIP && m == 3 && r >= 13) { if (hh == 0) s_p[drow(m, r, 0) * ST + j] = h[m][r]; }
+            else s_p[drow(m, r, hh) * ST + j] = h[m][r];
+        }
     __builtin_amdgcn_fence(__ATOMIC_ACQ_REL, "wavefront");
     __builtin_amdgcn_wave_barrier();
 }
@@ -515,13 +559,13 @@
 }
 #endif
 
-template <int INV, int NT, bool SAVEP>
-__device__ __forceinline__ void chunk_piped(const V2Args& a, const SpK& k, float* s_p, float* s_y, int c, int hh, int j, int rows,
+template <int INV, int NT, bool SAVEP, class AT>
+__device__ __forceinline__ void chunk_piped(const AT& a, const SpK& k, float* s_p, float* s_y, int c, int hh, int j, int rows,
                                             float& run, int& oob_local, int (&bins)[3], f32x16 (&h)[4], const BFrag& bf,
                                             TFrag (&ring)[RD], unsigned voff, int64_t b0) {
     Live<NT> g{h, bf, a.A2 + (size_t)(c + 1) * GBLK * 64, voff, ring};
     g.start();
-    chunk_to_lds(h, s_p, hh, j);
+    chunk_to_lds<AT::CLIP>(h, s_p, hh, j);
 #if BGK_V2_SAVE
     if constexpr (SAVEP) save_chunk_params(a, s_p, c, (int)threadIdx.x & 63, b0, rows);
 #endif
@@ -722,7 +766,7 @@
 
     const int nfs = a.nfs, ys = a.ys;
     const StageTiles stg{a.d_c, a.periodic, nfs, ys, a.stage, a.y_dma, d, a.magic_d, rows, lane};
-    stage_issue(stg, a.cs, b0, y_t, s_p, s_y);
+    if (!(BGK_V2_ABL & 1)) stage_issue(stg, a.cs, b0, y_t, s_p, s_y);
     f32x16 h[4], acc[4];
     TFrag ring[RD];
     BFrag bf;
@@ -833,6 +877,9 @@
         __builtin_amdgcn_fence(__ATOMIC_ACQ_REL, "wavefront");
         __builtin_amdgcn_wave_barrier();
     }
+#if BGK_V2_ABL & 2
+    if (a.B != -1) return;
+#endif
     if (hh == 0 && j < rows) {
         if (a.accumulate) a.dlogp[b0 + j] += run; else a.dlogp[b0 + j] = run;
     }
@@ -844,6 +891,177 @@
     V2_TS(5 + a.n_chunks);
   }
 }
+
+#if !BGK_V2_SAVE && !BGK_V2_BF16
+struct ChainLayer {
+    const uint4* A0; const uint4* A1; const uint4* A2; const float* cs_dev; int32_t* oob_count;
+    uint64_t circ_mask;
+    float c0, c1, c2;
+    int S0, d, d_c, periodic, n_chunks, last_tiles, tsel, nfs;
+    uint32_t magic_c;
+    SpC sc;
+};
+typedef const __attribute__((address_space(4))) ChainLayer* clayer_t;
+typedef const __attribute__((address_space(4))) float* cfloat_t;
+struct ChainArgs {
+    const ChainLayer* layers; int n_layers;
+    const float* in0; const float* in1; float* out0; float* out1;
+    int w0, w1; int64_t B; float* dlogp; int accumulate;
+    int off0, off1, spare, lds_per_wave;
+};
+
+template <int ACT, int INV>
+__global__ __launch_bounds__(FTHREADS, 2) void coupling_rqs_dense_h2v2_kernel_chain(ChainArgs a) {
+    asm volatile("s_setreg_imm32_b32 hwreg(HW_REG_MODE, 23, 1), 1");
+    extern __shared__ __attribute__((aligned(16))) float smem[];
+    const int wave = __builtin_amdgcn_readfirstlane((int)(threadIdx.x >> 6));
+    float* s_p = smem + (size_t)wave * a.lds_per_wave;
+    const int64_t n_tiles = (a.B + 31) / 32;
+    const int64_t tile = (int64_t)blockIdx.x * FW + wave;
+    if (tile >= n_tiles) return;
+    const int lane = (int)threadIdx.x & 63, j = lane & 31, hh = lane >> 5;
+    const unsigned voff = (unsigned)lane * 16u;
+    const int64_t b0 = tile * 32;
+    const int rows = (int)((a.B - b0) < 32 ? (a.B - b0) : 32);
+    const clayer_t layers = (clayer_t)a.layers;
+
+    const float dl_in = a.dlogp[b0 + (j < rows ? j : 0)];
+    dma_tile32(s_p + a.off0, a.in0 + b0 * a.w0, 32 * a.w0, rows * a.w0, lane);
+    dma_tile32(s_p + a.off1, a.in1 + b0 * a.w1, 32 * a.w1, rows * a.w1, lane);
+    TFrag ring[RD];
+    L0Frag fa;
+    l0_request(fa, layers->A0, 0, lane);
+    {
+        f32x16 acc[4];
+        BFrag bf;
+        Live<4> g{acc, bf, layers->A1, voff, ring};
+        g.start();
+    }
+    asm volatile("s_waitcnt vmcnt(0)" ::: "memory");
+    __builtin_amdgcn_fence(__ATOMIC_ACQ_REL, "wavefront");
+    __builtin_amdgcn_wave_barrier();
+    float total = a.accumulate ? dl_in : 0.0f;
+    asm volatile("" : "+v"(total));
+
+#pragma clang loop unroll(disable)
+    for (int li = 0; li < a.n_layers; ++li) {
+        const clayer_t L = layers + li;
+        f32x16 h[4], acc[4];
+        BFrag bf;
+        L0Frag fb;
+#pragma unroll
+        for (int m = 0; m < 4; ++m) { asm volatile("" : "=v"(fb.v[m][0])); asm volatile("" : "=v"(fb.v[m][1])); }
+        const int d = L->d, d_c = L->d_c, nfs = L->nfs, S0 = L->S0, n_chunks = L->n_chunks;
+        float c0 = L->c0, c1 = L->c1, c2 = L->c2;
+        const cfloat_t cs = (cfloat_t)L->cs_dev;
+        if (cs) { c0 = cs[1]; c1 = cs[3]; c2 = cs[5]; }
+        const int y_off = L->tsel ? a.off1 : a.off0;
+        float* s_y = s_p + y_off;
+        const float* s_c = s_p + (L->tsel ? a.off0 : a.off1);
+        const int n_in = L->periodic ? 2 * d_c : d_c;
+
+        const float* frow = s_c + j * nfs + 8 * hh;
+        if (L->periodic) {
+            const uint32_t magic_c = L->magic_c;
+            for (int i = lane; i < 32 * d_c; i += 64) {
+                const int r = (int)(__umul24((unsigned)i, magic_c) >> 20), c = i - (int)__umul24((unsigned)r, (unsigned)d_c);
+                float sv, cv;
+                v2_sincos2pi(s_c[i], &sv, &cv);
+                float* f = s_p + (int)__umul24((unsigned)r, (unsigned)nfs) + c;
+                f[0] = cv;
+                f[d_c] = sv;
+            }
+            __builtin_amdgcn_fence(__ATOMIC_ACQ_REL, "wavefront");
+            __builtin_amdgcn_wave_barrier();
+            frow = s_p + j * nfs + 8 * hh;
+        }
+
+#pragma unroll
+        for (int m = 0; m < 4; ++m)
+#pragma unroll
+            for (int r = 0; r < 16; ++r) h[m][r] = 0.0f;
+        {
+            const uint4* A0 = L->A0;
+            const int rel0 = 16 * (S0 - 1) + 8 * hh - n_in;
+            for (int s = 0; s < S0; s += 2) {
+                if (s + 1 < S0) l0_request(fb, A0, s + 1, lane);
+                l0_step(h, fa, frow + 16 * s, s + 1 == S0, rel0);
+                if (s + 1 < S0) {
+                    if (s + 2 < S0) l0_request(fa, A0, s + 2, lane);
+                    l0_step(h, fb, frow + 16 * (s + 1), s + 2 == S0, rel0);
+                }
+            }
+        }
+        {
+            Live<4> g{acc, bf, L->A1, voff, ring};
+            g.attach();
+            NoLive none;
+            act_split_tile<ACT, 0>(Hooks<NoLive, 0, 1>{none}, h[0], c0, bf);
+            __builtin_amdgcn_sched_barrier(0);
+            act_split_tile<ACT, 1>(Hooks<Live<4>, 0, 100>{g}, h[1], c0, bf);
+            act_split_tile<ACT, 2>(Hooks<Live<4>, 24, 100>{g}, h[2], c0, bf);
+            act_split_tile<ACT, 3>(Hooks<Live<4>, 48, 100>{g}, h[3], c0, bf);
+            __builtin_amdgcn_sched_barrier(0);
+            g.template events<(72 * Live<4>::NEV) / 100, Live<4>::NEV>();
+        }
+        float run = 0.0f;
+        int oob_local = 0;
+        {
+            Live<4> g{h, bf, L->A2, voff, ring};
+            g.start();
+            NoLive none;
+            act_split_tile<ACT, 0>(Hooks<NoLive, 0, 1>{none}, acc[0], c1, bf);
+            __builtin_amdgcn_sched_barrier(0);
+            act_split_tile<ACT, 1>(Hooks<Live<4>, 0, 100>{g}, acc[1], c1, bf);
+            act_split_tile<ACT, 2>(Hooks<Live<4>, 24, 100>{g}, acc[2], c1, bf);
+            act_split_tile<ACT, 3>(Hooks<Live<4>, 48, 100>{g}, acc[3], c1, bf);
+            __builtin_amdgcn_sched_barrier(0);
+            g.template events<(72 * Live<4>::NEV) / 100, Live<4>::NEV>();
+        }
+        CLArgs la;
+        la.A2 = L->A2; la.circ_mask = L->circ_mask; la.ys = d; la.spare = a.spare - y_off;
+        la.scp = &L->sc;
+        if constexpr (!INV) load_spc(la.sc, la.scp);
+        const SpK k{c2 * 1.44269504088896341f, c2 * L->sc.beta * 1.44269504088896341f, c2};
+        int bins[3] = {0, 0, 0};
+        for (int c = 0; c + 1 < n_chunks; ++c) {
+            if (c + 2 < n_chunks || L->last_tiles > 2) {
+                chunk_piped<INV, 4, false>(la, k, s_p, s_y, c, hh, j, rows, run, oob_local, bins, h, bf, ring, voff, b0);
+            } else {
+                chunk_piped<INV, 2, false>(la, k, s_p, s_y, c, hh, j, rows, run, oob_local, bins, h, bf, ring, voff, b0);
+            }
+            __builtin_amdgcn_fence(__ATOMIC_ACQ_REL, "wavefront");
+            __builtin_amdgcn_wave_barrier();
+        }
+        {
+            const int c = n_chunks - 1, nd = d - c * DPC;
+            const clayer_t N = layers + (li + 1 < a.n_layers ? li + 1 : li);
+            l0_request(fa, N->A0, 0, lane);
+            {
+                Live<4> g{acc, bf, N->A1, voff, ring};
+                g.start();
+            }
+            NoLive none;
+            chunk_to_lds<true>(h, s_p, hh, j);
+            spline_slot<INV, 0, 1>(none, la, k, s_p, s_y, c, nd, hh, j, rows, run, oob_local, bins);
+            if (nd > 2) spline_slot<INV, 1, 1>(none, la, k, s_p, s_y, c, nd, hh, j, rows, run, oob_local, bins);
+            if (nd > 4) spline_slot<INV, 2, 1>(none, la, k, s_p, s_y, c, nd, hh, j, rows, run, oob_local, bins);
+            __builtin_amdgcn_fence(__ATOMIC_ACQ_REL, "wavefront");
+            __builtin_amdgcn_wave_barrier();
+        }
+        total += run;
+        int32_t* oob_count = L->oob_count;
+        if (oob_count && __builtin_amdgcn_ballot_w64(oob_local != 0)) {
+            for (int off = 32; off > 0; off >>= 1) oob_local += __shfl_xor(oob_local, off);
+            if (lane == 0) atomicAdd(oob_count, oob_local);
+        }
+    }
+    if (hh == 0 && j < rows) a.dlogp[b0 + j] = total;
+    const int lane_st = (int)__builtin_amdgcn_mbcnt_hi(~0u, __builtin_amdgcn_mbcnt_lo(~0u, 0u));
+    if (a.out0) store_tile32(a.out0 + b0 * a.w0, a.w0, s_p + a.off0, a.w0, a.w0, 0u, rows, lane_st, 1);
+    if (a.out1) store_tile32(a.out1 + b0 * a.w1, a.w1, s_p + a.off1, a.w1, a.w1, 0u, rows, lane_st, 1);
+}
+#endif
 
 struct TilePlan { int nfs, ys, stage, y_dma, out_lin; };
 TilePlan plan_tiles(const CondSegs& cs, int d_c, int periodic, const float* y, int64_t ldy, const float* out, int64_t ldo, int d, int tile_floats) {
@@ -1507,6 +1725,73 @@
 }
 #endif
 
+#if !BGK_V2_SAVE && !BGK_V2_BF16 && !BGK_V2_AFFTRAIN
+int64_t bgk_rqs_chain_layer_size(void) { return (int64_t)sizeof(ChainLayer); }
+
+int bgk_fill_rqs_chain_layer(const char* what, void* table_host, int32_t index, int32_t transformed, int32_t w0, int32_t w1, int32_t periodic,
+                             const void* A0p, const void* A1p, const void* A2p, float c0, float c1, float c2, const float* cs_dev,
+                             int32_t H0, int32_t H1, int32_t K, uint64_t circ_mask, int32_t inverse,
+                             double left, double right, double bottom, double top,
+                             double min_bin_width, double min_bin_height, double min_derivative, int32_t identity_init, int32_t* oob_count) {
+    BGK_CHECK_ARG(table_host && index >= 0 && (transformed == 0 || transformed == 1) && A0p && A1p && A2p, "%s: bad arguments", what);
+    const int d = transformed ? w1 : w0, d_c = transformed ? w0 : w1;
+    const int n_in = periodic ? 2 * d_c : d_c;
+    const int nfs = periodic ? (n_in | 1) : d_c;
+    if (bgk_h2_variant != 2 || H0 != 128 || H1 != 128 || K != KB || w0 <= 0 || w1 <= 0 || d > 64 || (w0 & 7) == 0 || (w1 & 7) == 0
+        || 32 * (w0 + w1) > 5120 - DPC * PPD * ST - 32 || 32 * nfs + 16 > DPC * PPD * ST) {
+        bgk_set_error("%s: layer outside the chain kernel's envelope (H %d x %d, K %d, widths %d + %d)", what, H0, H1, K, w0, w1);
+        return BGK_EUNSUPPORTED;
+    }
+    ChainLayer l;
+    memset(&l, 0, sizeof(l));
+    l.A0 = reinterpret_cast<const uint4*>(A0p); l.A1 = reinterpret_cast<const uint4*>(A1p); l.A2 = reinterpret_cast<const uint4*>(A2p);
+    l.cs_dev = cs_dev; l.oob_count = oob_count; l.circ_mask = circ_mask;
+    l.c0 = c0; l.c1 = c1; l.c2 = c2;
+    l.S0 = (n_in + 1 + 15) / 16; l.d = d; l.d_c = d_c; l.periodic = periodic;
+    l.n_chunks = (d + DPC - 1) / DPC;
+    l.last_tiles = ((d - (l.n_chunks - 1) * DPC) * PPD + 31) / 32;
+    l.tsel = transformed; l.nfs = nfs; l.magic_c = magic_div(d_c);
+    l.sc.left = (float)left; l.sc.right = (float)right;
+    const SetK sw = make_set(left, right, min_bin_width, KB), sh = make_set(bottom, top, min_bin_height, KB);
+    l.sc.sa = inverse ? sw : sh;
+    l.sc.sb = inverse ? sh : sw;
+    const double beta = identity_init ? (0.6931471805599453 / (1.0 - min_derivative)) : 1.0;
+    l.sc.beta = (float)beta; l.sc.kout = (float)(0.6931471805599453 / (double)(float)beta); l.sc.min_d = (float)min_derivative;
+    memcpy(static_cast<char*>(table_host) + (size_t)index * sizeof(ChainLayer), &l, sizeof(l));
+    return 0;
+}
+
+int bgk_launch_rqs_dense_h2v2_chain(const char* what, const void* table_dev, int32_t n_layers, int32_t act, int32_t inverse,
+                                    const float* in0, const float* in1, int32_t w0, int32_t w1, float* out0, float* out1, int64_t B,
+                                    float* dlogp, int32_t accumulate, void* stream) {
+    BGK_CHECK_ARG(table_dev && n_layers >= 1 && in0 && in1 && dlogp && B > 0, "%s: bad arguments", what);
+    const auto al16 = [](const void* p) { return ((uintptr_t)p & 15) == 0; };
+    if (bgk_h2_variant != 2 || w0 <= 0 || w1 <= 0 || (w0 & 7) == 0 || (w1 & 7) == 0 || 32 * (w0 + w1) > 5120 - DPC * PPD * ST - 32
+        || !al16(in0) || !al16(in1) || !al16(out0) || !al16(out1) || !al16(table_dev)) {
+        bgk_set_error("%s: outside the chain kernel's envelope (widths %d + %d, 16-byte aligned contiguous fields)", what, w0, w1);
+        return BGK_EUNSUPPORTED;
+    }
+    ChainArgs a;
+    a.layers = static_cast<const ChainLayer*>(table_dev); a.n_layers = n_layers;
+    a.in0 = in0; a.in1 = in1; a.out0 = out0; a.out1 = out1; a.w0 = w0; a.w1 = w1; a.B = B; a.dlogp = dlogp; a.accumulate = accumulate;
+    a.off0 = DPC * PPD * ST; a.off1 = a.off0 + 32 * w0; a.spare = a.off1 + 32 * w1;
+    a.lds_per_wave = a.spare + 32;
+    const size_t shmem = sizeof(float) * (size_t)FW * a.lds_per_wave;
+    const int64_t n_wg = ((B + 31) / 32 + FW - 1) / FW;
+    BGK_CHECK_ARG(n_wg < (int64_t)0x7fffffff, "%s: batch too large for one launch", what);
+    const int grid = (int)n_wg;
+    hipStream_t st = (hipStream_t)stream;
+#define BGK_LAUNCH(A, I) do { (void)hipFuncSetAttribute(reinterpret_cast<const void*>(coupling_rqs_dense_h2v2_kernel_chain<A, I>), \
+                                                       hipFuncAttributeMaxDynamicSharedMemorySize, 160 * 1024); \
+                              hipLaunchKernelGGL((coupling_rqs_dense_h2v2_kernel_chain<A, I>), dim3(grid), dim3(FTHREADS), shmem, st, a); } while (0)
+    if (act == 1) { if (inverse) BGK_LAUNCH(1, 1); else BGK_LAUNCH(1, 0); }
+    else if (act == 2) { if (inverse) BGK_LAUNCH(2, 1); else BGK_LAUNCH(2, 0); }
+    else { if (inverse) BGK_LAUNCH(3, 1); else BGK_LAUNCH(3, 0); }
+#undef BGK_LAUNCH
+    return bgk_launch_status(what);
+}
+#endif
+
 #if !BGK_V2_SAVE && !BGK_V2_BF16
 #if BGK_V2_AFFTRAIN
 int bgk_launch_affine_dense_v2_train(const BgkAffTrainSave* save,
diff --git a/bgflow_amd/dense.py b/bgflow_amd/dense.py
--- a/bgflow_amd/dense.py
+++ b/bgflow_amd/dense.py
@@ -1068,6 +1068,77 @@
     return res + (bins,) if want_bin_idx else res
 
 
+def spline_chain_infer(blocks, xs, inverse, acc, store):
+    first = blocks[0]
+    s0, s1 = sorted((int(first.transformed_indices[0]), int(first.cond_indices[0])))
+    if max(s0, s1) >= len(xs):
+        return None
+    f0, f1 = xs[s0], xs[s1]
+    for f in (f0, f1):
+        if not (torch.is_tensor(f) and f.is_cuda and f.dtype == torch.float32 and f.dim() == 2 and f.is_contiguous()
+                and f.data_ptr() % 16 == 0):
+            return None
+    B = f0.shape[0]
+    if B == 0 or f1.shape[0] != B or f1.device != f0.device or not acc.buf.is_cuda or acc.buf.shape[0] != B:
+        return None
+    dev = f0.device
+    widths = (f0.shape[1], f1.shape[1])
+    lib = _lib.lib()
+    key, act, written = [dev, bool(inverse)], None, [False, False]
+    for block in blocks:
+        tr = block.transformer
+        t = 0 if int(block.transformed_indices[0]) == s0 else 1
+        if tr.return_bin_indices or not tr.allow_fused:
+            return None
+        _, nc_host = tr._nc_slot(widths[t], dev)
+        plan = _fused_plan(tr, widths[t], nc_host)
+        if plan is None or plan["mode"] != "f16x2" or plan.get("deep") or plan["hidden"] != 128 or plan["n_bins"] != 8 \
+                or plan.get("cs") is None or plan["d_c"] != widths[1 - t] or plan["packed"][0].device != dev:
+            return None
+        if act is not None and plan["act"] != act:
+            return None
+        act = plan["act"]
+        written[t] = True
+        A0, A1, A2, (c0, c1, c2) = plan["packed"]
+        st = tr._default_settings
+        key.append((t, widths[0], widths[1], int(plan["periodic"]), A0.data_ptr(), A1.data_ptr(), A2.data_ptr(), c0, c1, c2,
+                    plan["cs"].data_ptr(), 128, 128, 8, plan["circ_mask"], int(inverse),
+                    float(tr._left), float(tr._right), float(tr._bottom), float(tr._top),
+                    st["min_bin_width"], st["min_bin_height"], st["min_derivative"], int(st.get("enable_identity_init", False)),
+                    tr._oob_counter(dev).data_ptr()))
+    key = tuple(key)
+    if store.get("key") != key:
+        size = int(lib.bgk_coupling_rqs_chain_layer_size())
+        host = torch.zeros(len(blocks) * size, dtype=torch.uint8)
+        for i, args in enumerate(key[2:]):
+            status = lib.bgk_coupling_rqs_chain_layer(host.data_ptr(), i, *args)
+            if status == -2:
+                store.clear()
+                store.update(key=key, table=None)
+                return None
+            _lib.check(status, "bgk_coupling_rqs_chain_layer")
+        store.clear()
+        store.update(key=key, table=host.to(dev))
+    table = store["table"]
+    if table is None:
+        return None
+    _lib.require_hip(f0, f1)
+    outs = [torch.empty_like(f) if w else None for f, w in zip((f0, f1), written)]
+    dlogp, accumulate = acc.peek()
+    with torch.cuda.device(dev):
+        status = lib.bgk_coupling_rqs_dense_h2_chain(_lib.ptr(table), len(blocks), act, int(inverse), _lib.ptr(f0), _lib.ptr(f1),
+                                                     widths[0], widths[1], _lib.ptr(outs[0]), _lib.ptr(outs[1]), B,
+                                                     _lib.ptr(dlogp), int(bool(accumulate)), _lib.stream_ptr(dev))
+    if status == -2:
+        return None
+    _lib.check(status, "bgk_coupling_rqs_dense_h2_chain")
+    acc.commit()
+    ys = list(xs)
+    ys[s0] = outs[0] if outs[0] is not None else f0
+    ys[s1] = outs[1] if outs[1] is not None else f1
+    return ys
+
+
 def _act_fwd_bwd(code):
     if code == 1:
         return torch.nn.functional.silu, lambda g, z, h: torch.ops.aten.silu_backward(g, z)
diff --git a/bgflow_amd/flow.py b/bgflow_amd/flow.py
--- a/bgflow_amd/flow.py
+++ b/bgflow_amd/flow.py
@@ -122,6 +122,7 @@
     FUSE_COUPLING_STACKS = True
     FUSE_TRAINING_CHAINS = True
     FUSE_CONSTANT_MERGE = True
+    FUSE_INFERENCE_CHAINS = True
 
     _bgk_acc = True
     ACCUMULATE_IN_KERNELS = True
@@ -186,17 +187,40 @@
                         *xs, ddlogp = seg(*xs, inverse=inverse, **kwargs)
                 total = ddlogp if total is None else total + ddlogp
             return (*xs, 0.0 if total is None else total)
+        chains = {}
+        if self.FUSE_INFERENCE_CHAINS and not set(kwargs) - {"temperature"}:
+            chains = dict(self.inference_chains(inverse=inverse))
         kwargs[ACC_KW] = acc
-        for i, (label, seg) in enumerate(self.segments(inverse=inverse)):
-            kw = _acc_kwargs(seg, kwargs)
+        segs = self.segments(inverse=inverse)
+
+        def step(i, xs):
+            end = chains.get(i)
+            if end is not None:
+                from .dense import spline_chain_infer
+                store = self._segment_cache.setdefault(("chain tables", bool(inverse), i), {})
+                ys = spline_chain_infer([seg for _, seg in segs[i:end]], xs, inverse, acc, store)
+                if ys is not None:
+                    return ys, end
+                del chains[i]
+            seg = segs[i][1]
+            *ys, ddlogp = seg(*xs, inverse=inverse, **_acc_kwargs(seg, kwargs))
+            acc.add(ddlogp)
+            return ys, i + 1
+        i = 0
+        while i < len(segs):
             if around is None:
-                *xs, ddlogp = seg(*xs, inverse=inverse, **kw)
-                acc.add(ddlogp)
+                xs, i = step(i, xs)
             else:
-                with around(i, label):
-                    *xs, ddlogp = seg(*xs, inverse=inverse, **kw)
-                    acc.add(ddlogp)
+                with around(i, segs[i][0]):
+                    xs, i = step(i, xs)
         return (*xs, acc if outer is not None else acc.result())
+
+    def inference_chains(self, inverse=False):
+        segs = self.segments(inverse=inverse)
+        key = ("chains", bool(inverse))
+        if key not in self._segment_cache:
+            self._segment_cache[key] = _inference_chains(segs)
+        return self._segment_cache[key]
 
     def segments(self, inverse=False, train=False):
         blocks = list(self._blocks)
@@ -295,6 +319,25 @@
             return self._blocks[index]
         picked = np.arange(len(self))[index]
         return SequentialFlow([self._blocks[i] for i in picked])
+
+
+def _inference_chains(segs):
+    from .transformer import ConditionalSplineTransformer
+    out, start, slots = [], None, None
+
+    def close(end):
+        if start is not None and end - start >= 2:
+            out.append((start, end))
+    for i, (_, seg) in enumerate(segs):
+        ok = type(seg) is CouplingFlow and type(seg.transformer) is ConditionalSplineTransformer and seg.cat_dim == -1 \
+            and len(seg.transformed_indices) == 1 and len(seg.cond_indices) == 1
+        pair = frozenset((int(seg.transformed_indices[0]), int(seg.cond_indices[0]))) if ok else None
+        if ok and start is not None and pair == slots:
+            continue
+        close(i)
+        start, slots = (i, pair) if ok else (None, None)
+    close(len(segs))
+    return out
 
 
 def _with_train_chains(segs):
diff --git a/include/bgflow_amd.h b/include/bgflow_amd.h
--- a/include/bgflow_amd.h
+++ b/include/bgflow_amd.h
@@ -163,6 +163,18 @@
                               int32_t identity_init,
                               float* out, int64_t ldo, float* dlogp, int32_t accumulate,
                               int32_t* bin_idx, int32_t* oob_count, void* stream);
+
+int64_t bgk_coupling_rqs_chain_layer_size(void);
+int bgk_coupling_rqs_chain_layer(void* table_host, int32_t index, int32_t transformed, int32_t w0, int32_t w1, int32_t periodic,
+                                 const void* A0p, const void* A1p, const void* A2p,
+                                 float c0, float c1, float c2, const float* cs_dev,
+                                 int32_t H0, int32_t H1, int32_t K, uint64_t circ_mask, int32_t inverse,
+                                 double left, double right, double bottom, double top,
+                                 double min_bin_width, double min_bin_height, double min_derivative,
+                                 int32_t identity_init, int32_t* oob_count);
+int bgk_coupling_rqs_dense_h2_chain(const void* table_dev, int32_t n_layers, int32_t act, int32_t inverse,
+                                    const float* in0, const float* in1, int32_t w0, int32_t w1,
+                                    float* out0, float* out1, int64_t B, float* dlogp, int32_t accumulate, void* stream);
 
 int bgk_coupling_rqs_dense_deep(const float* cond, int64_t ldc, int32_t d_c, int32_t periodic,
                                 const void* A0p, const void* A1p, const void* A2p, float c0, const float* c1s, float c2,
```

Result: no change. 134.1 million, median of 6 (+0.6%).
